# pedrocr/imagepipe

Hardware: AMD Instinct MI355X
Metric: megapixels/sec full raw->sRGB pipe, 100 MP f32 frame (higher is better)
Workload: dtype f32

## Files before the change

### bindings/rust/imagepipe_amd_sys.rs

```rust
#![allow(non_camel_case_types, dead_code)]
use std::os::raw::{c_char, c_int, c_uint, c_void};

pub const IPK_OK: c_int = 0;
pub const IPK_NOOP: c_int = 1;
pub const IPK_ERR_NOT_INIT: c_int = -1;
pub const IPK_ERR_INVALID: c_int = -2;
pub const IPK_ERR_HIP: c_int = -3;
pub const IPK_ERR_NO_DEVICE: c_int = -4;
pub const IPK_ERR_UNSUPPORTED: c_int = -5;
pub const IPK_ERR_NOMEM: c_int = -6;

pub const IPK_OR_NORMAL: c_int = 0;
pub const IPK_OR_HFLIP: c_int = 1;
pub const IPK_OR_ROT180: c_int = 2;
pub const IPK_OR_VFLIP: c_int = 3;
pub const IPK_OR_TRANSPOSE: c_int = 4;
pub const IPK_OR_ROT90: c_int = 5;
pub const IPK_OR_TRANSVERSE: c_int = 6;
pub const IPK_OR_ROT270: c_int = 7;
pub const IPK_OR_UNKNOWN: c_int = 8;

pub const IPK_ROT_NORMAL: c_int = 0;
pub const IPK_ROT_90: c_int = 1;
pub const IPK_ROT_180: c_int = 2;
// ... 167 lines not shown
  pub fn ipk_tolab(src4: *const f32, width: usize, height: usize, monochrome: c_int, wb_coeffs: *const f32, cam_to_xyz_normalized: *const f32, dst3: *mut f32, stream: *mut c_void) -> c_int;
  pub fn ipk_basecurve(src3: *const f32, width: usize, height: usize, exposure: f32, points: *const f32, npoints: c_int, dst3: *mut f32, stream: *mut c_void) -> c_int;
  pub fn ipk_fromlab(src3: *const f32, width: usize, height: usize, dst3: *mut f32, stream: *mut c_void) -> c_int;
  pub fn ipk_gamma(src: *const f32, width: usize, height: usize, colors: usize, linear: c_int, dst: *mut f32, stream: *mut c_void) -> c_int;
  pub fn ipk_rotate_buffer(src3: *const f32, width: usize, height: usize, orientation: c_int, dst3: *mut f32, out_width: *mut usize, out_height: *mut usize, stream: *mut c_void) -> c_int;
  pub fn ipk_rotate_image_u8(src3: *const u8, width: usize, height: usize, orientation: c_int, dst3: *mut u8, out_width: *mut usize, out_height: *mut usize, stream: *mut c_void) -> c_int;
  pub fn ipk_rotate_image_u16(src3: *const u16, width: usize, height: usize, orientation: c_int, dst3: *mut u16, out_width: *mut usize, out_height: *mut usize, stream: *mut c_void) -> c_int;
  pub fn ipk_transform(src3: *const f32, width: usize, height: usize, rotation: c_int, fliph: c_int, flipv: c_int, dst3: *mut f32, out_width: *mut usize, out_height: *mut usize, stream: *mut c_void) -> c_int;
  pub fn ipk_output8bit(src: *const f32, n: usize, dst: *mut u8, stream: *mut c_void) -> c_int;
  pub fn ipk_output16bit(src: *const f32, n: usize, dst: *mut u16, stream: *mut c_void) -> c_int;
  pub fn ipk_raw_to_srgb(p: *const IpkFusedParams, src: *const c_void, dst: *mut c_void, stream: *mut c_void) -> c_int;
  pub fn ipk_raw_to_srgb_batch(p: *const IpkFusedParams, srcs: *const *const c_void, dsts: *const *mut c_void, n: usize, stream: *mut c_void) -> c_int;
  pub fn ipk_raw_to_srgb_oriented(p: *const IpkFusedParams, src: *const c_void, orientation: c_int, dst: *mut c_void, out_width: *mut usize, out_height: *mut usize, stream: *mut c_void) -> c_int;
  pub fn ipk_raw_to_srgb_resampled(p: *const IpkFusedParams, src: *const c_void, tlx: i64, tly: i64, trx: i64, try_: i64, blx: i64, bly: i64, nwidth: usize, nheight: usize, dst: *mut c_void, stream: *mut c_void) -> c_int;
  pub fn ipk_raw_to_srgb_scaled(p: *const IpkFusedParams, src: *const c_void, nwidth: usize, nheight: usize, dst: *mut c_void, stream: *mut c_void) -> c_int;
  pub fn ipk_raw_to_srgb_resampled_window(p: *const IpkFusedParams, src: *const c_void, tlx: i64, tly: i64, trx: i64, try_: i64, blx: i64, bly: i64, nwidth: usize, nheight: usize, wx: usize, wy: usize, ww: usize, wh: usize, dst: *mut c_void, stream: *mut c_void) -> c_int;
  pub fn ipk_raw_to_srgb_scaled_window(p: *const IpkFusedParams, src: *const c_void, nwidth: usize, nheight: usize, wx: usize, wy: usize, ww: usize, wh: usize, dst: *mut c_void, stream: *mut c_void) -> c_int;
  pub fn ipk_transform_window_footprint(width: usize, height: usize, tlx: i64, tly: i64, trx: i64, try_: i64, blx: i64, bly: i64, nwidth: usize, nheight: usize, wx: usize, wy: usize, ww: usize, wh: usize, out4: *mut usize) -> c_int;
  pub fn ipk_pointwise_chain(src4: *const f32, width: usize, height: usize, monochrome: c_int, wb_coeffs: *const f32, cam_to_xyz_normalized: *const f32, exposure: f32, points: *const f32, npoints: c_int, linear: c_int, dst3: *mut f32, stream: *mut c_void) -> c_int;
  pub fn ipk_pointwise_chain_out(src4: *const f32, width: usize, height: usize, monochrome: c_int, wb_coeffs: *const f32, cam_to_xyz_normalized: *const f32, exposure: f32, points: *const f32, npoints: c_int, linear: c_int, out_type: c_int, dst: *mut c_void, stream: *mut c_void) -> c_int;
  pub fn ipk_raster_to_srgb(src: *const c_void, src_type: c_int, width: usize, height: usize, wb_coeffs: *const f32, cam_to_xyz_normalized: *const f32, exposure: f32, points: *const f32, npoints: c_int, linear: c_int, out_type: c_int, dst: *mut c_void, stream: *mut c_void) -> c_int;
  pub fn ipk_pipeline_sizes(d: *const IpkPipelineDesc, demosaic_w: *mut usize, demosaic_h: *mut usize, final_w: *mut usize, final_h: *mut usize) -> c_int;
  pub fn ipk_pipeline_run(d: *const IpkPipelineDesc, src: *const c_void, dst: *mut c_void, out_type: c_int, used_fused: *mut c_int, stream: *mut c_void) -> c_int;
  pub fn ipk_pipeline_takes_fastpath(d: *const IpkPipelineDesc, out_type: c_int) -> c_int;
  pub fn ipk_pipeline_fuses_rotatecrop(d: *const IpkPipelineDesc, out_type: c_int) -> c_int;
  pub fn ipk_pipeline_fuses_scaledown(d: *const IpkPipelineDesc, out_type: c_int) -> c_int;
  pub fn ipk_pipeline_fuses_four_colour(d: *const IpkPipelineDesc, out_type: c_int) -> c_int;
  pub fn ipk_timing_begin() -> c_int;
  pub fn ipk_timing_end(out: *mut IpkStageTime, max_stages: c_int, n_stages: *mut c_int) -> c_int;
  pub fn ipk_host_pipeline_run(d: *const IpkPipelineDesc, src: *const c_void, dst: *mut c_void, out_type: c_int, used_fused: *mut c_int) -> c_int;
  pub fn ipk_pipeline_region(d: *const IpkPipelineDesc, out_type: c_int, x: usize, y: usize, w: usize, h: usize, src_x: *mut usize, src_y: *mut usize, src_w: *mut usize, src_h: *mut usize) -> c_int;
  pub fn ipk_pipeline_run_region(d: *const IpkPipelineDesc, src: *const c_void, x: usize, y: usize, w: usize, h: usize, dst: *mut c_void, out_type: c_int, windowed: *mut c_int, stream: *mut c_void) -> c_int;
  pub fn ipk_host_pipeline_run_region(d: *const IpkPipelineDesc, src: *const c_void, x: usize, y: usize, w: usize, h: usize, dst: *mut c_void, out_type: c_int, windowed: *mut c_int) -> c_int;
  pub fn ipk_host_pipeline_run_batch(d: *const IpkPipelineDesc, srcs: *const *const c_void, dsts: *const *mut c_void, n: usize, out_type: c_int, used_fused: *mut c_int) -> c_int;
  pub fn ipk_pipeline_run_batch(d: *const IpkPipelineDesc, srcs: *const *const c_void, dsts: *const *mut c_void, n: usize, out_type: c_int, used_fused: *mut c_int, stream: *mut c_void) -> c_int;
  pub fn ipk_pipeline_run_batch_multi(d: *const IpkPipelineDesc, srcs: *const *const c_void, dsts: *const *mut c_void, n: usize, out_type: c_int, used_fused: *mut c_int) -> c_int;
  pub fn ipk_devices_sync() -> c_int;
  pub fn ipk_host_pipeline_run_batch_multi(d: *const IpkPipelineDesc, srcs: *const *const c_void, dsts: *const *mut c_void, n: usize, out_type: c_int, used_fused: *mut c_int) -> c_int;
  pub fn ipk_host_alloc(bytes: usize) -> *mut c_void;
  pub fn ipk_host_free(p: *mut c_void);
  pub fn ipk_pipeline_hashes(d: *const IpkPipelineDesc, out_type: c_int, source_id: u64, out256: *mut u8) -> c_int;
  pub fn ipk_cache_new(max_bytes: usize, out: *mut *mut IpkCache) -> c_int;
  pub fn ipk_cache_free(cache: *mut IpkCache) -> c_int;
  pub fn ipk_cache_clear(cache: *mut IpkCache) -> c_int;
  pub fn ipk_cache_contains(cache: *const IpkCache, key32: *const u8) -> c_int;
  pub fn ipk_cache_stats(cache: *const IpkCache, bytes: *mut usize, entries: *mut usize, hits: *mut u64, misses: *mut u64, evictions: *mut u64) -> c_int;
  pub fn ipk_cache_get(cache: *mut IpkCache, key32: *const u8, data: *mut *const f32, width: *mut usize, height: *mut usize, colors: *mut usize, monochrome: *mut c_int) -> c_int;
  pub fn ipk_pipeline_run_cached(d: *const IpkPipelineDesc, src: *const c_void, source_id: u64, cache: *mut IpkCache, out_type: c_int, dst: *mut c_void, ops_run: *mut c_int, used_fused: *mut c_int, stream: *mut c_void) -> c_int;
  pub fn ipk_band_plan(height: usize, nranks: c_int, cfa_period: c_int, bands: *mut IpkBand) -> c_int;
  pub fn ipk_band_plan_scaled(height: usize, nheight: usize, nranks: c_int, bands: *mut IpkBand) -> c_int;
  pub fn ipk_raw_scaled_demosaic_band(src: *const c_void, src_type: c_int, owidth: usize, x: usize, width: usize, height: usize, black0: f32, white0: f32, cfa: *const c_char, nwidth: usize, nheight: usize, band: *const IpkBand, dst4: *mut f32, stream: *mut c_void) -> c_int;
  pub fn ipk_comm_unique_id(id128: *mut u8) -> c_int;
  pub fn ipk_comm_init_rccl(id128: *const u8, rank: c_int, nranks: c_int, out: *mut *mut IpkComm) -> c_int;
  pub fn ipk_comm_init_host(rank: c_int, nranks: c_int, exchange: IpkExchangeFn, ctx: *mut c_void, out: *mut *mut IpkComm) -> c_int;
  pub fn ipk_comm_free(comm: *mut IpkComm) -> c_int;
  pub fn ipk_comm_info(comm: *const IpkComm, rank: *mut c_int, nranks: *mut c_int, transport: *mut c_int) -> c_int;
  pub fn ipk_band_exchange_halo(comm: *mut IpkComm, slab: *mut c_void, row_bytes: usize, bands: *const IpkBand, stream: *mut c_void) -> c_int;
  pub fn ipk_host_band_exchange_halo(comm: *mut IpkComm, slab: *mut c_void, row_bytes: usize, bands: *const IpkBand) -> c_int;
  pub fn ipk_band_gather(comm: *mut IpkComm, frame: *mut c_void, out_row_bytes: usize, bands: *const IpkBand, root: c_int, stream: *mut c_void) -> c_int;
  pub fn ipk_host_band_gather(comm: *mut IpkComm, frame: *mut c_void, out_row_bytes: usize, bands: *const IpkBand, root: c_int) -> c_int;
  pub fn ipk_band_gather_begin(comm: *mut IpkComm, frame: *mut c_void, out_row_bytes: usize, bands: *const IpkBand, root: c_int, after_stream: *mut c_void) -> c_int;
  pub fn ipk_comm_wait(comm: *mut IpkComm, stream: *mut c_void) -> c_int;
  pub fn ipk_comm_selftest(comm: *mut IpkComm) -> c_int;
  pub fn ipk_host_gofloat_cfa_u16(src: *const u16, owidth: usize, oheight: usize, x: usize, y: usize, width: usize, height: usize, black0: f32, white0: f32, dst: *mut f32) -> c_int;
  pub fn ipk_host_gofloat_cfa_f32(src: *const f32, owidth: usize, oheight: usize, x: usize, y: usize, width: usize, height: usize, black0: f32, white0: f32, dst: *mut f32) -> c_int;
  pub fn ipk_host_demosaic_full(src: *const f32, width: usize, height: usize, cfa: *const c_char, dst4: *mut f32) -> c_int;
  pub fn ipk_host_transform_buffer_f32(src: *const f32, width: usize, height: usize, tlx: i64, tly: i64, trx: i64, try_: i64, blx: i64, bly: i64, nwidth: usize, nheight: usize, components: usize, cfa: *const c_char, dst: *mut f32) -> c_int;
  pub fn ipk_host_tolab(src4: *const f32, width: usize, height: usize, monochrome: c_int, wb_coeffs: *const f32, cam_to_xyz_normalized: *const f32, dst3: *mut f32) -> c_int;
  pub fn ipk_host_basecurve(src3: *const f32, width: usize, height: usize, exposure: f32, points: *const f32, npoints: c_int, dst3: *mut f32) -> c_int;
  pub fn ipk_host_fromlab(src3: *const f32, width: usize, height: usize, dst3: *mut f32) -> c_int;
  pub fn ipk_host_gamma(src: *const f32, width: usize, height: usize, colors: usize, linear: c_int, dst: *mut f32) -> c_int;
  pub fn ipk_host_rotate_buffer(src3: *const f32, width: usize, height: usize, orientation: c_int, dst3: *mut f32, out_width: *mut usize, out_height: *mut usize) -> c_int;
  pub fn ipk_host_output8bit(src: *const f32, n: usize, dst: *mut u8) -> c_int;
  pub fn ipk_host_output16bit(src: *const f32, n: usize, dst: *mut u16) -> c_int;
  pub fn ipk_host_raw_to_srgb(p: *const IpkFusedParams, src: *const c_void, dst: *mut c_void) -> c_int;
  pub fn ipk_selftest_cdiv(c: f32, variant: c_int, lo: f32, hi: f32, include_special: c_int, n_bad: *mut u64, first_bad_bits: *mut u32) -> c_int;
  pub fn ipk_selftest_lut_weight(n_bad: *mut u64, first_bad_bits: *mut u32) -> c_int;
  pub fn ipk_selftest_clamp01(n_bad: *mut u64, first_bad_bits: *mut u32) -> c_int;
  pub fn ipk_copy_probe(src: *const c_void, dst: *mut c_void, bytes: usize, stream: *mut c_void) -> c_int;
  pub fn ipk_mix_probe(src: *const c_void, dst: *mut c_void, src_bytes: usize, stream: *mut c_void) -> c_int;
  pub fn ipk_clock_probe(out2_dev: *mut u64, spin_us: u32, stream: *mut c_void) -> c_int;
  pub fn ipk_stream_probe(p: *const IpkFusedParams, src: *const c_void, dst: *mut c_void, stream: *mut c_void) -> c_int;
  pub fn ipk_selftest_spline3(exposure: f32, points: *const f32, npoints: c_int, n_bad: *mut u64, first_bad_bits: *mut u32) -> c_int;
  pub fn ipk_selftest_quant8(variant: c_int, n_bad: *mut u64, first_bad_bits: *mut u32) -> c_int;
  pub fn ipk_selftest_q8(n_bad: *mut u64, first_bad_bits: *mut u32) -> c_int;
  pub fn ipk_selftest_quant16(n_bad: *mut u64, first_bad_bits: *mut u32) -> c_int;
  pub fn ipk_selftest_cbrtf(r#in: *const f32, out: *mut f32, n: usize, variant: c_int, stream: *mut c_void) -> c_int;
  pub fn ipk_selftest_task_queue(enabled: c_int) -> c_int;
  pub fn ipk_selftest_launch_log(enabled: c_int) -> c_int;
  pub fn ipk_selftest_launch_log_read(buf: *mut c_char, cap: usize) -> usize;
  pub fn ipk_selftest_cache_put(cache: *mut IpkCache, key32: *const u8, bytes: usize) -> c_int;
  pub fn ipk_selftest_sha256(data: *const c_void, n: usize, out32: *mut u8) -> c_int;
}
```

### imagepipe_amd/_lib.py

```python
import ctypes as C
import os

_HERE = os.path.dirname(os.path.abspath(__file__))
SO_PATH = os.environ.get("IPK_SO_OVERRIDE") or os.path.join(_HERE, "libimagepipe_amd.so")

IPK_OK, IPK_NOOP = 0, 1
SRC_U16, SRC_F32, SRC_RGB8, SRC_RGB16 = 0, 1, 2, 3
OUT_F32, OUT_U8, OUT_U16 = 0, 1, 2
SCHED_AUTO, SCHED_SPLIT = 0, 1
FUSED_ON, FUSED_FOUR_COLOUR, FUSED_WINDOW_REGIONS = 1, 2, 4
OR_NORMAL, OR_HFLIP, OR_ROT180, OR_VFLIP, OR_TRANSPOSE, OR_ROT90, OR_TRANSVERSE, OR_ROT270, OR_UNKNOWN = range(9)
ROT_NORMAL, ROT_90, ROT_180, ROT_270 = range(4)

_sz = C.c_size_t
_vp = C.c_void_p
_fp = C.POINTER(C.c_float)
_szp = C.POINTER(C.c_size_t)
_i64 = C.c_int64


class _SizedDesc(C.Structure):

    def __init__(self, *a, **k):
        super().__init__(*a, **k)
# ... 73 lines not shown
    "ipk_orientation_to_flips": (C.c_int, [C.c_int, C.POINTER(C.c_int)]),
    "ipk_orientation_from_flips": (C.c_int, [C.c_int, C.c_int, C.c_int]),
    "ipk_transform_orientation": (C.c_int, [C.c_int, C.c_int, C.c_int]),
    "ipk_gofloat_cfa_u16": (C.c_int, [_vp] + _GO + [C.c_float, C.c_float, _vp, _vp]),
    "ipk_gofloat_cfa_f32": (C.c_int, [_vp] + _GO + [C.c_float, C.c_float, _vp, _vp]),
    "ipk_gofloat_mono_u16": (C.c_int, [_vp] + _GO + [C.c_float, C.c_float, _vp, _vp]),
    "ipk_gofloat_mono_f32": (C.c_int, [_vp] + _GO + [C.c_float, C.c_float, _vp, _vp]),
    "ipk_gofloat_rgb_u16": (C.c_int, [_vp] + _GO + [_fp, _fp, _vp, _vp]),
    "ipk_gofloat_rgb_f32": (C.c_int, [_vp] + _GO + [_fp, _fp, _vp, _vp]),
    "ipk_gofloat_other_u8": (C.c_int, [_vp] + _GO + [_vp, _vp]),
    "ipk_gofloat_other_u16": (C.c_int, [_vp] + _GO + [_vp, _vp]),
    "ipk_demosaic_full": (C.c_int, [_vp, _sz, _sz, C.c_char_p, _vp, _vp]),
    "ipk_demosaic_full_band": (C.c_int, [_vp, _sz, _sz, _sz, _sz, _sz, _sz, C.c_char_p, _vp, _vp]),
    "ipk_transform_buffer_f32": (C.c_int, [_vp, _sz, _sz] + _CORNERS + [_sz, _sz, _sz, C.c_char_p, _vp, _vp]),
    "ipk_transform_buffer_u8": (C.c_int, [_vp, _sz, _sz] + _CORNERS + [_sz, _sz, _sz, C.c_char_p, _vp, _vp]),
    "ipk_transform_buffer_u16": (C.c_int, [_vp, _sz, _sz] + _CORNERS + [_sz, _sz, _sz, C.c_char_p, _vp, _vp]),
    "ipk_scaled_demosaic": (C.c_int, [_vp, _sz, _sz, C.c_char_p, _sz, _sz, _vp, _vp]),
    "ipk_scale_down_opbuf": (C.c_int, [_vp, _sz, _sz, _sz, _sz, _vp, _vp]),
    "ipk_raw_scaled_demosaic": (C.c_int, [_vp, C.c_int, _sz, _sz, _sz, _sz, _sz, C.c_float, C.c_float, C.c_char_p, _sz, _sz, _vp, _vp]),
    "ipk_raster_scale_down": (C.c_int, [_vp, C.c_int, _sz, _sz, _sz, _sz, _sz, _sz, _sz, _vp, _vp]),
    "ipk_demosaic_run": (C.c_int, [_vp, _sz, _sz, _sz, C.c_char_p, _sz, _sz, _vp, _szp, _szp, _vp]),
    "ipk_rotatecrop": (C.c_int, [_vp, _sz, _sz, _sz, _fp, _vp, _szp, _szp, _vp]),
    "ipk_tolab": (C.c_int, [_vp, _sz, _sz, C.c_int, _fp, _fp, _vp, _vp]),
    "ipk_basecurve": (C.c_int, [_vp, _sz, _sz, C.c_float, _fp, C.c_int, _vp, _vp]),
    "ipk_fromlab": (C.c_int, [_vp, _sz, _sz, _vp, _vp]),
    "ipk_gamma": (C.c_int, [_vp, _sz, _sz, _sz, C.c_int, _vp, _vp]),
    "ipk_rotate_buffer": (C.c_int, [_vp, _sz, _sz, C.c_int, _vp, _szp, _szp, _vp]),
    "ipk_rotate_image_u8": (C.c_int, [_vp, _sz, _sz, C.c_int, _vp, _szp, _szp, _vp]),
    "ipk_rotate_image_u16": (C.c_int, [_vp, _sz, _sz, C.c_int, _vp, _szp, _szp, _vp]),
    "ipk_transform": (C.c_int, [_vp, _sz, _sz, C.c_int, C.c_int, C.c_int, _vp, _szp, _szp, _vp]),
    "ipk_output8bit": (C.c_int, [_vp, _sz, _vp, _vp]),
    "ipk_output16bit": (C.c_int, [_vp, _sz, _vp, _vp]),
    "ipk_raw_to_srgb": (C.c_int, [C.POINTER(FusedParams), _vp, _vp, _vp]),
    "ipk_raw_to_srgb_batch": (C.c_int, [C.POINTER(FusedParams), C.POINTER(C.c_void_p), C.POINTER(C.c_void_p), _sz, _vp]),
    "ipk_raw_to_srgb_oriented": (C.c_int, [C.POINTER(FusedParams), _vp, C.c_int, _vp, _szp, _szp, _vp]),
    "ipk_raw_to_srgb_resampled": (C.c_int, [C.POINTER(FusedParams), _vp] + _CORNERS + [_sz, _sz, _vp, _vp]),
    "ipk_raw_to_srgb_scaled": (C.c_int, [C.POINTER(FusedParams), _vp, _sz, _sz, _vp, _vp]),
    "ipk_raw_to_srgb_resampled_window": (C.c_int, [C.POINTER(FusedParams), _vp] + _CORNERS + [_sz, _sz, _sz, _sz, _sz, _sz, _vp, _vp]),
    "ipk_raw_to_srgb_scaled_window": (C.c_int, [C.POINTER(FusedParams), _vp, _sz, _sz, _sz, _sz, _sz, _sz, _vp, _vp]),
    "ipk_transform_window_footprint": (C.c_int, [_sz, _sz] + _CORNERS + [_sz, _sz, _sz, _sz, _sz, _sz, _szp]),
    "ipk_pipeline_sizes": (C.c_int, [C.POINTER(PipelineDesc), _szp, _szp, _szp, _szp]),
    "ipk_pipeline_run": (C.c_int, [C.POINTER(PipelineDesc), _vp, _vp, C.c_int, C.POINTER(C.c_int), _vp]),
    "ipk_host_pipeline_run": (C.c_int, [C.POINTER(PipelineDesc), _vp, _vp, C.c_int, C.POINTER(C.c_int)]),
    "ipk_pipeline_region": (C.c_int, [C.POINTER(PipelineDesc), C.c_int, _sz, _sz, _sz, _sz, _szp, _szp, _szp, _szp]),
    "ipk_pipeline_run_region": (C.c_int, [C.POINTER(PipelineDesc), _vp, _sz, _sz, _sz, _sz, _vp, C.c_int, C.POINTER(C.c_int), _vp]),
    "ipk_host_pipeline_run_region": (C.c_int, [C.POINTER(PipelineDesc), _vp, _sz, _sz, _sz, _sz, _vp, C.c_int, C.POINTER(C.c_int)]),
    "ipk_host_pipeline_run_batch": (C.c_int, [C.POINTER(PipelineDesc), C.POINTER(_vp), C.POINTER(_vp), _sz, C.c_int, C.POINTER(C.c_int)]),
    "ipk_pipeline_run_batch": (C.c_int, [C.POINTER(PipelineDesc), C.POINTER(_vp), C.POINTER(_vp), _sz, C.c_int, C.POINTER(C.c_int), _vp]),
    "ipk_pipeline_run_batch_multi": (C.c_int, [C.POINTER(PipelineDesc), C.POINTER(_vp), C.POINTER(_vp), _sz, C.c_int, C.POINTER(C.c_int)]),
    "ipk_host_pipeline_run_batch_multi": (C.c_int, [C.POINTER(PipelineDesc), C.POINTER(_vp), C.POINTER(_vp), _sz, C.c_int, C.POINTER(C.c_int)]),
    "ipk_devices_sync": (C.c_int, []),
    "ipk_ctx_create": (C.c_int, [C.c_int, C.POINTER(_vp)]),
    "ipk_ctx_destroy": (C.c_int, [_vp]),
    "ipk_ctx_make_current": (C.c_int, [_vp]),
    "ipk_ctx_current": (_vp, []),
    "ipk_ctx_device": (C.c_int, [_vp]),
    "ipk_init_devices": (C.c_int, [C.POINTER(C.c_int), C.c_int]),
    "ipk_device_set_size": (C.c_int, []),
    "ipk_device_ctx": (_vp, [C.c_int]),
    "ipk_deal_frames": (C.c_int, [_sz, C.c_int, C.c_int, _szp, _szp, _szp]),
    "ipk_host_alloc": (_vp, [_sz]),
    "ipk_host_free": (None, [_vp]),
    "ipk_host_gofloat_cfa_u16": (C.c_int, [_vp, _sz, _sz, _sz, _sz, _sz, _sz, C.c_float, C.c_float, _vp]),
    "ipk_host_gofloat_cfa_f32": (C.c_int, [_vp, _sz, _sz, _sz, _sz, _sz, _sz, C.c_float, C.c_float, _vp]),
    "ipk_host_demosaic_full": (C.c_int, [_vp, _sz, _sz, C.c_char_p, _vp]),
    "ipk_host_transform_buffer_f32": (C.c_int, [_vp, _sz, _sz] + _CORNERS + [_sz, _sz, _sz, C.c_char_p, _vp]),
    "ipk_host_tolab": (C.c_int, [_vp, _sz, _sz, C.c_int, _fp, _fp, _vp]),
    "ipk_host_basecurve": (C.c_int, [_vp, _sz, _sz, C.c_float, _fp, C.c_int, _vp]),
    "ipk_host_fromlab": (C.c_int, [_vp, _sz, _sz, _vp]),
    "ipk_host_gamma": (C.c_int, [_vp, _sz, _sz, _sz, C.c_int, _vp]),
    "ipk_host_rotate_buffer": (C.c_int, [_vp, _sz, _sz, C.c_int, _vp, _szp, _szp]),
    "ipk_host_output8bit": (C.c_int, [_vp, _sz, _vp]),
    "ipk_host_output16bit": (C.c_int, [_vp, _sz, _vp]),
    "ipk_host_raw_to_srgb": (C.c_int, [C.POINTER(FusedParams), _vp, _vp]),
    "ipk_selftest_cdiv": (C.c_int, [C.c_float, C.c_int, C.c_float, C.c_float, C.c_int, C.POINTER(C.c_uint64), C.POINTER(C.c_uint32)]),
    "ipk_selftest_lut_weight": (C.c_int, [C.POINTER(C.c_uint64), C.POINTER(C.c_uint32)]),
    "ipk_selftest_clamp01": (C.c_int, [C.POINTER(C.c_uint64), C.POINTER(C.c_uint32)]),
    "ipk_abi_sizeof": (_sz, [C.c_int]),
    "ipk_copy_probe": (C.c_int, [_vp, _vp, _sz, _vp]),
    "ipk_mix_probe": (C.c_int, [_vp, _vp, _sz, _vp]),
    "ipk_clock_probe": (C.c_int, [_vp, C.c_uint32, _vp]),
    "ipk_stream_probe": (C.c_int, [C.POINTER(FusedParams), _vp, _vp, _vp]),
    "ipk_selftest_spline3": (C.c_int, [C.c_float, _fp, C.c_int, C.POINTER(C.c_uint64), C.POINTER(C.c_uint32)]),
    "ipk_selftest_quant8": (C.c_int, [C.c_int, C.POINTER(C.c_uint64), C.POINTER(C.c_uint32)]),
    "ipk_selftest_q8": (C.c_int, [C.POINTER(C.c_uint64), C.POINTER(C.c_uint32)]),
    "ipk_selftest_quant16": (C.c_int, [C.POINTER(C.c_uint64), C.POINTER(C.c_uint32)]),
    "ipk_selftest_cbrtf": (C.c_int, [_vp, _vp, _sz, C.c_int, _vp]),
    "ipk_selftest_task_queue": (C.c_int, [C.c_int]),
    "ipk_selftest_launch_log": (C.c_int, [C.c_int]),
    "ipk_selftest_launch_log_read": (_sz, [C.c_char_p, _sz]),
    "ipk_selftest_cache_put": (C.c_int, [_vp, C.c_char_p, _sz]),
    "ipk_selftest_sha256": (C.c_int, [C.c_char_p, _sz, C.c_char_p]),
    "ipk_pointwise_chain": (C.c_int, [_vp, _sz, _sz, C.c_int, _fp, _fp, C.c_float, _fp, C.c_int, C.c_int, _vp, _vp]),
    "ipk_pointwise_chain_out": (C.c_int, [_vp, _sz, _sz, C.c_int, _fp, _fp, C.c_float, _fp, C.c_int, C.c_int, C.c_int, _vp, _vp]),
    "ipk_raster_to_srgb": (C.c_int, [_vp, C.c_int, _sz, _sz, _fp, _fp, C.c_float, _fp, C.c_int, C.c_int, C.c_int, _vp, _vp]),
    "ipk_pipeline_takes_fastpath": (C.c_int, [C.POINTER(PipelineDesc), C.c_int]),
    "ipk_pipeline_fuses_rotatecrop": (C.c_int, [C.POINTER(PipelineDesc), C.c_int]),
    "ipk_pipeline_fuses_scaledown": (C.c_int, [C.POINTER(PipelineDesc), C.c_int]),
    "ipk_pipeline_fuses_four_colour": (C.c_int, [C.POINTER(PipelineDesc), C.c_int]),
    "ipk_pipeline_hashes": (C.c_int, [C.POINTER(PipelineDesc), C.c_int, C.c_uint64, C.c_char_p]),
    "ipk_cache_new": (C.c_int, [_sz, C.POINTER(C.c_void_p)]),
    "ipk_cache_free": (C.c_int, [_vp]),
    "ipk_cache_clear": (C.c_int, [_vp]),
    "ipk_cache_contains": (C.c_int, [_vp, C.c_char_p]),
    "ipk_cache_stats": (C.c_int, [_vp, C.POINTER(_sz), C.POINTER(_sz), C.POINTER(C.c_uint64), C.POINTER(C.c_uint64), C.POINTER(C.c_uint64)]),
    "ipk_cache_get": (C.c_int, [_vp, C.c_char_p, C.POINTER(C.c_void_p), C.POINTER(_sz), C.POINTER(_sz), C.POINTER(_sz), C.POINTER(C.c_int)]),
    "ipk_timing_begin": (C.c_int, []),
    "ipk_timing_end": (C.c_int, [C.POINTER(StageTime), C.c_int, C.POINTER(C.c_int)]),
    "ipk_band_plan": (C.c_int, [_sz, C.c_int, C.c_int, _bp]),
    "ipk_band_plan_scaled": (C.c_int, [_sz, _sz, C.c_int, _bp]),
    "ipk_raw_scaled_demosaic_band": (C.c_int, [_vp, C.c_int, _sz, _sz, _sz, _sz, C.c_float, C.c_float, C.c_char_p, _sz, _sz, _bp, _vp, _vp]),
    "ipk_comm_unique_id": (C.c_int, [C.c_char_p]),
    "ipk_comm_init_rccl": (C.c_int, [C.c_char_p, C.c_int, C.c_int, C.POINTER(_vp)]),
    "ipk_comm_init_host": (C.c_int, [C.c_int, C.c_int, EXCHANGE_FN, _vp, C.POINTER(_vp)]),
    "ipk_comm_free": (C.c_int, [_vp]),
    "ipk_comm_info": (C.c_int, [_vp, C.POINTER(C.c_int), C.POINTER(C.c_int), C.POINTER(C.c_int)]),
    "ipk_band_exchange_halo": (C.c_int, [_vp, _vp, _sz, _bp, _vp]),
    "ipk_host_band_exchange_halo": (C.c_int, [_vp, _vp, _sz, _bp]),
    "ipk_band_gather": (C.c_int, [_vp, _vp, _sz, _bp, C.c_int, _vp]),
    "ipk_host_band_gather": (C.c_int, [_vp, _vp, _sz, _bp, C.c_int]),
    "ipk_band_gather_begin": (C.c_int, [_vp, _vp, _sz, _bp, C.c_int, _vp]),
    "ipk_comm_wait": (C.c_int, [_vp, _vp]),
    "ipk_comm_selftest": (C.c_int, [_vp]),
    "ipk_pipeline_run_cached": (C.c_int, [C.POINTER(PipelineDesc), _vp, C.c_uint64, _vp, C.c_int, _vp, C.POINTER(C.c_int), C.POINTER(C.c_int), _vp]),
}

_lib = None


class IpkError(RuntimeError):
    code = None


def load():
    global _lib
    if _lib is not None:
        return _lib
    if not os.path.exists(SO_PATH):
        raise ImportError(
            "imagepipe_amd: %s is missing -- build it with `python -c 'import __graft_entry__ as g; g.build()'` "
            "or `make -C imagepipe_amd/csrc`. There is no CPU fallback." % SO_PATH)
    lib = C.CDLL(SO_PATH, mode=C.RTLD_GLOBAL)
    for name, (res, args) in SIGNATURES.items():
        if os.environ.get("IPK_SO_OVERRIDE") and not hasattr(lib, name):
            continue
        fn = getattr(lib, name)
        fn.restype = res
        fn.argtypes = args
    _lib = lib
    return lib


def check(rc, what=""):
    if rc < 0:
        err = IpkError("%s failed (%d): %s" % (what or "ipk call", rc, load().ipk_last_error().decode()))
        err.code = rc
        raise err
    return rc
```

### imagepipe_amd/csrc/ipk_api.cpp

```cpp
#include <hip/hip_runtime_api.h>

#include <algorithm>
#include <cmath>
#include <cstdarg>
#include <cstdio>
#include <cstddef>
#include <cstring>
#include <atomic>
#include <map>
#include <memory>
#include <mutex>
#include <string>
#include <thread>
#include <vector>

#include "../../include/imagepipe_amd.h"
#include "ipk_hash.hpp"
#include "ipk_host.hpp"
#include "ipk_internal.hpp"
#include "ipk_launch.hpp"

namespace {

thread_local char g_err[512] = "";
// ... 1166 lines not shown
  return resampled_launch(p, src, corners, nwidth, nheight, dst, stream, "resampled", kResampledRefusal, &win);
}
int ipk_raw_to_srgb_scaled_window(const ipk_fused_params *p, const void *src, size_t nwidth, size_t nheight, size_t wx, size_t wy, size_t ww, size_t wh,
                                  void *dst, void *stream) {
  const ipk::ResampleWindow win = {wy, wx, wh, ww};
  return resampled_launch(p, src, nullptr, nwidth, nheight, dst, stream, "scaled", kScaledRefusal, &win);
}
int ipk_transform_window_footprint(size_t width, size_t height, int64_t tlx, int64_t tly, int64_t trx, int64_t try_, int64_t blx, int64_t bly,
                                   size_t nwidth, size_t nheight, size_t wx, size_t wy, size_t ww, size_t wh, size_t *out4) {
  if (!out4) return fail(IPK_ERR_INVALID, "null argument");
  ipk::ResamplePlan plan;
  if (!ipk::resample_skips(width, height, tlx, tly, trx, try_, blx, bly, nwidth, nheight, plan))
    return fail(IPK_ERR_UNSUPPORTED, "not a transform the fused paths take (output sides >= 2, finite skips, sides below 2^24)");
  if (ww == 0 || wh == 0 || wx > nwidth || ww > nwidth - wx || wy > nheight || wh > nheight - wy)
    return fail(IPK_ERR_INVALID, "window (%zu, %zu) %zux%zu is empty or outside the %zux%zu result", wx, wy, ww, wh, nwidth, nheight);
  const ipk::ResampleFootprint f = ipk::resample_footprint(plan, width, height, wy, wx, wh, ww);
  out4[0] = f.x; out4[1] = f.y; out4[2] = f.w; out4[3] = f.h;
  return IPK_OK;
}

static int selftest_collect(void *dev, uint64_t *n_bad, uint32_t *first_bad) {
  struct { unsigned long long bad; unsigned int first; unsigned int pad; } h;
  HIPCHK(hipMemcpy(&h, dev, sizeof(h), hipMemcpyDeviceToHost));
  (void)hipFree(dev);
  *n_bad = h.bad; if (first_bad) *first_bad = h.first;
  return IPK_OK;
}
static int selftest_alloc(void **dev) {
  struct { unsigned long long bad; unsigned int first; unsigned int pad; } h = {0, 0xFFFFFFFFu, 0};
  HIPCHK(hipMalloc(dev, sizeof(h)));
  HIPCHK(hipMemcpy(*dev, &h, sizeof(h), hipMemcpyHostToDevice));
  return IPK_OK;
}
int ipk_selftest_cdiv(float c, int variant, float lo, float hi, int include_special, uint64_t *n_bad, uint32_t *first_bad_bits) {
  REQUIRE_INIT();
  if (!(c > 0.0f) || variant < 0 || variant > 2 || !n_bad) return fail(IPK_ERR_INVALID, "bad selftest arguments");
  uint32_t lo_bits, hi_bits; std::memcpy(&lo_bits, &lo, 4); std::memcpy(&hi_bits, &hi, 4);
  void *dev; int rc = selftest_alloc(&dev); if (rc) return rc;
  ipk::launch_selftest_cdiv(c, variant, lo_bits, hi_bits, include_special, dev, nullptr);
  HIPCHK(hipGetLastError());
  return selftest_collect(dev, n_bad, first_bad_bits);
}
int ipk_selftest_lut_weight(uint64_t *n_bad, uint32_t *first_bad_bits) {
  REQUIRE_INIT();
  void *dev; int rc = selftest_alloc(&dev); if (rc) return rc;
  ipk::launch_selftest_fract(dev, nullptr); HIPCHK(hipGetLastError());
  return selftest_collect(dev, n_bad, first_bad_bits);
}
int ipk_selftest_clamp01(uint64_t *n_bad, uint32_t *first_bad_bits) {
  REQUIRE_INIT();
  void *dev; int rc = selftest_alloc(&dev); if (rc) return rc;
  ipk::launch_selftest_clamp(dev, nullptr); HIPCHK(hipGetLastError());
  return selftest_collect(dev, n_bad, first_bad_bits);
}
int ipk_copy_probe(const void *src, void *dst, size_t bytes, void *stream) {
  REQUIRE_INIT();
  if (!src || !dst || (bytes & 15) || ((uintptr_t)src & 15) || ((uintptr_t)dst & 15)) return fail(IPK_ERR_INVALID, "ipk_copy_probe wants 16-byte aligned buffers and a multiple of 16 bytes");
  ipk::launch_copy_probe(src, dst, bytes, cx().num_cus, S(stream)); HIPCHK(hipGetLastError());
  return IPK_OK;
}
int ipk_mix_probe(const void *src, void *dst, size_t src_bytes, void *stream) {
  REQUIRE_INIT();
  if (!src || !dst || (src_bytes & 4095) || ((uintptr_t)src & 15) || ((uintptr_t)dst & 15)) return fail(IPK_ERR_INVALID, "ipk_mix_probe wants 16-byte aligned buffers and a multiple of 4096 source bytes (whole blocks)");
  ipk::launch_mix_probe(src, dst, src_bytes, S(stream)); HIPCHK(hipGetLastError());
  return IPK_OK;
}
int ipk_clock_probe(uint64_t *out2_dev, uint32_t spin_us, void *stream) {
  REQUIRE_INIT();
  if (!out2_dev || spin_us == 0 || spin_us > 2000000u) return fail(IPK_ERR_INVALID, "ipk_clock_probe: null output or a spin outside (0, 2 s]");
  ipk::launch_clock_probe(out2_dev, (unsigned long long)spin_us * 100ull, S(stream)); HIPCHK(hipGetLastError());
  return IPK_OK;
}
int ipk_selftest_launch_log(int enabled) { ipk::launch_log_enable(enabled != 0); return IPK_OK; }
size_t ipk_selftest_launch_log_read(char *buf, size_t cap) { return ipk::launch_log_read(buf, cap); }
int ipk_selftest_task_queue(int enabled) { REQUIRE_INIT(); ipk::selftest_task_queue(enabled != 0); return IPK_OK; }
int ipk_selftest_spline3(float exposure, const float *points, int npoints, uint64_t *n_bad, uint32_t *first_bad_bits) {
  REQUIRE_INIT();
  if (!n_bad || (npoints > 0 && !points)) return fail(IPK_ERR_INVALID, "bad selftest arguments");
  ipk::Spline sp; int rc = build_curve(exposure, points, npoints, sp); if (rc) return rc;
  void *dev; rc = selftest_alloc(&dev); if (rc) return rc;
  if (ipk::launch_selftest_spline3(sp, dev, nullptr) != 0) { (void)hipFree(dev); return fail(IPK_ERR_UNSUPPORTED, "the kernels keep the select form for this curve"); }
  HIPCHK(hipGetLastError());
  return selftest_collect(dev, n_bad, first_bad_bits);
}
int ipk_selftest_quant16(uint64_t *n_bad, uint32_t *first_bad_bits) {
  REQUIRE_INIT();
  if (!n_bad) return fail(IPK_ERR_INVALID, "bad selftest arguments");
  void *dev; int rc = selftest_alloc(&dev); if (rc) return rc;
  ipk::launch_selftest_quant16(dev, nullptr); HIPCHK(hipGetLastError());
  return selftest_collect(dev, n_bad, first_bad_bits);
}
int ipk_selftest_q8(uint64_t *n_bad, uint32_t *first_bad_bits) {
  REQUIRE_INIT();
  if (!n_bad) return fail(IPK_ERR_INVALID, "bad selftest arguments");
  void *dev; int rc = selftest_alloc(&dev); if (rc) return rc;
  ipk::launch_selftest_q8(cx().lut_pairs[ipk::kLutGamma], cx().lut_q8, dev, nullptr); HIPCHK(hipGetLastError());
  return selftest_collect(dev, n_bad, first_bad_bits);
}
int ipk_selftest_quant8(int variant, uint64_t *n_bad, uint32_t *first_bad_bits) {
  REQUIRE_INIT();
  void *dev; int rc = selftest_alloc(&dev); if (rc) return rc;
  ipk::launch_selftest_quant8(dev, variant, nullptr); HIPCHK(hipGetLastError());
  return selftest_collect(dev, n_bad, first_bad_bits);
}
int ipk_selftest_cbrtf(const float *in, float *out, size_t n, int variant, void *stream) {
  REQUIRE_INIT();
  if (!in || !out || variant < 0 || variant > 5 || (variant >= 3 && n % 256 != 0)) return fail(IPK_ERR_INVALID, "bad selftest arguments");
  ipk::launch_selftest_cbrt(in, out, n, variant, cx().lut_pairs[ipk::kLutXyzLab], S(stream)); HIPCHK(hipGetLastError());
  return IPK_OK;
}

static ipk::RotateCrop rotatecrop_of(const ipk_pipeline_desc *d) {
  ipk::RotateCrop rc;
  rc.crop_top = d->rotatecrop[0]; rc.crop_right = d->rotatecrop[1]; rc.crop_bottom = d->rotatecrop[2];
  rc.crop_left = d->rotatecrop[3]; rc.rotation = d->rotatecrop[4];
  return rc;
}
static int pipeline_sizes_impl(const ipk_pipeline_desc *d, size_t *demosaic_w, size_t *demosaic_h, size_t *final_w, size_t *final_h,
                               ipk::RotateCrop *rc_state) {
  if (!d) return fail(IPK_ERR_INVALID, "null descriptor");
  if (d->rotation < 0 || d->rotation > 3) return fail(IPK_ERR_INVALID, "bad rotation");
  ipk::RotateCrop rc = rotatecrop_of(d);
  ipk::Rect r;
  if (!ipk::size_image(d->crop_top, d->crop_right, d->crop_bottom, d->crop_left, d->width, d->height, r))
    return fail(IPK_ERR_INVALID, "source smaller than 10x10");
  size_t w = r.width, h = r.height;
  rc.transform_forward(w, h, w, h);
  ipk::transform_forward(d->rotation, w, h, w, h);
  const ipk::Scaling s = ipk::calculate_scaling_total(w, h, d->maxwidth, d->maxheight);
  w = s.width; h = s.height;
  ipk::transform_forward(d->rotation, w, h, w, h);
  rc.transform_reverse(w, h, w, h);
  if (rc_state) *rc_state = rc;
  *demosaic_w = w; *demosaic_h = h;
  size_t pw = r.width, ph = r.height;
  if (ipk::calculate_scaling_total(pw, ph, w, h).scale > 1.0f) { pw = w; ph = h; }
  {
    int64_t pts[6]; size_t nw, nh;
    if (rotatecrop_of(d).corners(pw, ph, pts, nw, nh)) { pw = nw; ph = nh; }
  }
  {
    bool transpose, fx, fy;
    ipk::orientation_to_flips(ipk::transform_orientation(d->rotation, d->fliph != 0, d->flipv != 0), transpose, fx, fy);
    if (transpose) std::swap(pw, ph);
  }
  *final_w = pw; *final_h = ph;
  return IPK_OK;
}
int ipk_pipeline_sizes(const ipk_pipeline_desc *d, size_t *demosaic_w, size_t *demosaic_h, size_t *final_w, size_t *final_h) {
  IPK_FOLD_CFA(ipk_pipeline_desc, d)
  return pipeline_sizes_impl(d, demosaic_w, demosaic_h, final_w, final_h, nullptr);
}

static bool default_ops_other(const ipk_pipeline_desc *d) {
  auto same = [](float a, float b) { return std::memcmp(&a, &b, 4) == 0; };
  if (d->src_type != IPK_SRC_RGB8 && d->src_type != IPK_SRC_RGB16) return false;
  if (d->crop_top || d->crop_right || d->crop_bottom || d->crop_left || d->is_cfa || d->cfa[0]) return false;
  for (int i = 0; i < 4; ++i) if (!same(d->blacklevels[i], 0.0f) || !same(d->whitelevels[i], 0.0f)) return false;
  for (int i = 0; i < 5; ++i) if (!same(d->rotatecrop[i], 0.0f)) return false;
  float m[12]; ipk::srgb_d65_43(m);
  for (int i = 0; i < 12; ++i) if (!same(d->cam_to_xyz_normalized[i], m[i])) return false;
  const float wb[4] = {1.0f, 1.0f, 1.0f, 0.0f};
  for (int i = 0; i < 4; ++i) if (!same(d->wb_coeffs[i], wb[i])) return false;
  if (!same(d->exposure, 0.0f) || d->npoints != 0) return false;
  return d->rotation == 0 && !d->fliph && !d->flipv;
}
// ... 1015 lines not shown
```

### imagepipe_amd/csrc/ipk_device.hpp

```cpp
#pragma once
#include <hip/hip_runtime.h>
#include <stdint.h>

namespace ipkd {

typedef float2 LutPair;
constexpr int kLutPairs = 8192;
constexpr float kLutMaxF = 8191.0f;

constexpr float kWhiteX = 0.95047f, kWhiteY = 1.000f, kWhiteZ = 1.08883f;
constexpr float kLabE = 216.0f / 24389.0f;
constexpr float kLabK = 24389.0f / 27.0f;

__device__ __forceinline__ float rs_min(float a, float b) { return fminf(a, b); }
__device__ __forceinline__ float rs_max(float a, float b) { return fmaxf(a, b); }
__device__ __forceinline__ uint32_t f32_as_u32_sat(float f) { return __float2uint_rz(f); }

__device__ __forceinline__ LutPair lut_pair_at(const LutPair *__restrict__ tab, uint32_t key) { return tab[key]; }
__device__ __forceinline__ LutPair lut_pair_at(const float *__restrict__ tab, uint32_t key) {
  const float v1 = tab[key], v2 = tab[key + 1];
  return make_float2(v1, v2 - v1);
}
template <typename Tab>
__device__ __forceinline__ float lut_interp(const Tab *__restrict__ tab, float val) {
// ... 138 lines not shown
__device__ __forceinline__ uint32_t q8_sample(const Q8Entry *__restrict__ tab, float c ) {
  const Q8Entry e = tab[f32_as_u32_sat(c * kLutMaxF)];
  return e.k + (c >= e.t ? 1u : 0u);
}

__device__ __forceinline__ uint8_t output8bit_literal(float v) {
  return (uint8_t)f32_as_u32_sat(rs_min(rs_max(v * 256.0f, 0.0f), 255.0f));
}
__device__ __forceinline__ uint8_t output8bit(float v) { return output8bit_literal(v); }
__device__ __forceinline__ uint32_t output8bit_x4(float a, float b, float c, float d) {
  uint32_t w = __builtin_amdgcn_cvt_pk_u8_f32(floorf(a * 256.0f), 0u, 0u);
  w = __builtin_amdgcn_cvt_pk_u8_f32(floorf(b * 256.0f), 1u, w);
  w = __builtin_amdgcn_cvt_pk_u8_f32(floorf(c * 256.0f), 2u, w);
  return __builtin_amdgcn_cvt_pk_u8_f32(floorf(d * 256.0f), 3u, w);
}
__device__ __forceinline__ uint16_t output16bit_literal(float v) {
  return (uint16_t)f32_as_u32_sat(rs_min(rs_max(roundf(v * 65535.0f), 0.0f), 65535.0f));
}
__device__ __forceinline__ uint32_t output16bit_x2(float a, float b) {
  typedef unsigned short u16x2 __attribute__((ext_vector_type(2)));
  const u16x2 p = __builtin_amdgcn_cvt_pk_u16(f32_as_u32_sat(floorf(a * 65535.0f + 0.5f)), f32_as_u32_sat(floorf(b * 65535.0f + 0.5f)));
  return (uint32_t)p.x | ((uint32_t)p.y << 16);
}
__device__ __forceinline__ uint16_t output16bit(float v) { return (uint16_t)(output16bit_x2(v, 0.0f) & 0xFFFFu); }
__device__ __forceinline__ float input8bit(uint8_t v) { return (float)v / 255.0f; }
__device__ __forceinline__ float input16bit(uint16_t v) { return (float)v / 65535.0f; }

constexpr int kSplineMaxKnots = 66;
constexpr int kKnotSegRec = 5 * kSplineMaxKnots + 2;
constexpr int kKnotFloats = kKnotSegRec + 16;
struct SplineDev {
  int npoints, nseg;
  float px[kSplineMaxKnots], py[kSplineMaxKnots], c1[kSplineMaxKnots], c2[kSplineMaxKnots], c3[kSplineMaxKnots];
  int grid_ok; float grid_scale, grid_xl, grid_yl;
};
__device__ __forceinline__ float spline_poly(float y, float c1, float c2, float c3, float diff) {
  return y + c1 * diff + c2 * diff * diff + c3 * diff * diff * diff;
}
__device__ __forceinline__ float spline_interpolate(const SplineDev &s, float val) {
  const int np = s.npoints;
  if (np == 2) {
    if (val >= s.px[1]) return s.py[1];
    if (!(val > s.px[0])) return s.py[0];
    return spline_poly(s.py[0], s.c1[0], s.c2[0], s.c3[0], val - s.px[0]);
  }
  if (np == 3) {
    if (val >= s.px[2]) return s.py[2];
    if (!(val > s.px[0])) return s.py[0];
    const float x1 = s.px[1];
    if (x1 < val) return spline_poly(s.py[1], s.c1[1], s.c2[1], s.c3[1], val - x1);
    if (x1 > val) return spline_poly(s.py[0], s.c1[0], s.c2[0], s.c3[0], val - s.px[0]);
    return s.py[1];
  }
  if (val >= s.px[np - 1]) return s.py[np - 1];
  if (val <= s.px[0]) return s.py[0];
  int low = 0, high = s.nseg - 1;
  while (low <= high) {
    const int mid = (low + high) / 2;
    const float xhere = s.px[mid];
    if (xhere < val) low = mid + 1;
    else if (xhere > val) high = mid - 1;
    else return s.py[mid];
  }
  const int i = high > 0 ? high : 0;
  return spline_poly(s.py[i], s.c1[i], s.c2[i], s.c3[i], val - s.px[i]);
}

__device__ __forceinline__ float spline_interpolate_lds(const float *__restrict__ t, int np, int nseg, float val) {
  const float *px = t, *py = t + kSplineMaxKnots, *c1 = t + 2 * kSplineMaxKnots, *c2 = t + 3 * kSplineMaxKnots, *c3 = t + 4 * kSplineMaxKnots;
  if (val >= px[np - 1]) return py[np - 1];
  if (val <= px[0]) return py[0];
  int low = 0, high = nseg - 1;
  while (low <= high) {
    const int mid = (low + high) / 2;
    const float xhere = px[mid];
    if (xhere < val) low = mid + 1;
    else if (xhere > val) high = mid - 1;
    else return py[mid];
  }
  const int i = high > 0 ? high : 0;
  return spline_poly(py[i], c1[i], c2[i], c3[i], val - px[i]);
}

__device__ __forceinline__ float spline_interpolate_3a(const SplineDev &s, const float *__restrict__ lds_knots, float val) {
  const float x0 = s.px[0], x1 = s.px[1], x2 = s.px[2];
  const float v1 = fmaxf(val, x0);
  const bool up = v1 >= x1;
  const float *rec = lds_knots + kKnotSegRec + (up ? 8 : 0);
  const float4 q = *reinterpret_cast<const float4 *>(rec);
  const float r = spline_poly(q.y, q.z, q.w, rec[4], v1 - q.x);
  return (val >= x2) ? s.py[2] : r;
}
__device__ __forceinline__ float spline_interpolate_sel(const SplineDev &s, const float *__restrict__ lds_knots, float val) {
  const int np = s.npoints;
  if (np == 3) {
    const float x0 = s.px[0], x1 = s.px[1], x2 = s.px[2];
    const bool up = x1 < val, down = x1 > val;
    const int i = up ? 1 : 0;
    const float bx = lds_knots[i], by = lds_knots[kSplineMaxKnots + i];
    const float k1 = lds_knots[2 * kSplineMaxKnots + i], k2 = lds_knots[3 * kSplineMaxKnots + i], k3 = lds_knots[4 * kSplineMaxKnots + i];
    float r = spline_poly(by, k1, k2, k3, val - bx);
    r = (!up && !down) ? s.py[1] : r;
    r = !(val > x0) ? s.py[0] : r;
    r = (val >= x2) ? s.py[2] : r;
    return r;
  }
  if (np == 2) {
    float r = spline_poly(s.py[0], s.c1[0], s.c2[0], s.c3[0], val - s.px[0]);
    r = !(val > s.px[0]) ? s.py[0] : r;
    r = (val >= s.px[1]) ? s.py[1] : r;
    return r;
  }
  return spline_interpolate_lds(lds_knots, np, s.nseg, val);
}

constexpr int kGridCells = 256;
constexpr int kGridFloats = 2 * kGridCells + 8 * kSplineMaxKnots;
__device__ __host__ inline uint32_t spline_grid_cell(float v1, float x0, float scale) {
  const float t = (v1 - x0) * scale;
#if defined(__HIP_DEVICE_COMPILE__)
  const uint32_t c = __float2uint_rz(t);
#else
  const uint32_t c = !(t < 4294967296.0f) ? 0xFFFFFFFFu : (uint32_t)t;
#endif
  return c < (uint32_t)(kGridCells - 1) ? c : (uint32_t)(kGridCells - 1);
}
__device__ __forceinline__ void fill_grid(float *__restrict__ g, const SplineDev &s, int t) {
  if (t >= kGridCells) return;
  const float x0 = s.px[0];
  uint32_t base = 0u; float nx = __builtin_inff();
  for (int k = 1; k < s.nseg; ++k) {
    const uint32_t ck = spline_grid_cell(s.px[k], x0, s.grid_scale);
    if (ck < (uint32_t)t) base = (uint32_t)k;
    else if (ck == (uint32_t)t) nx = s.px[k];
  }
  g[2 * t] = __uint_as_float((2u * kGridCells + 8u * base) * 4u);
  g[2 * t + 1] = nx;
  if (t < s.nseg) {
    float *r = g + 2 * kGridCells + 8 * t;
    r[0] = s.px[t]; r[1] = s.py[t]; r[2] = s.c1[t]; r[3] = s.c2[t]; r[4] = s.c3[t]; r[5] = 0.0f; r[6] = 0.0f; r[7] = 0.0f;
  }
}
__device__ __forceinline__ float spline_interpolate_grid(const SplineDev &s, const float *__restrict__ g, float val) {
  const float x0 = s.px[0];
  const float v1 = fmaxf(val, x0);
  const uint32_t c = spline_grid_cell(v1, x0, s.grid_scale);
  const float2 ce = reinterpret_cast<const float2 *>(g)[c];
  const uint32_t off = __float_as_uint(ce.x) + (ce.y <= v1 ? 32u : 0u);
  const float *rec = reinterpret_cast<const float *>(reinterpret_cast<const char *>(g) + off);
  const float4 q = *reinterpret_cast<const float4 *>(rec);
  const float r = spline_poly(q.y, q.z, q.w, rec[4], v1 - q.x);
  return (val >= s.grid_xl) ? s.grid_yl : r;
}

__device__ __forceinline__ void fill_knots(float *__restrict__ lds, const SplineDev &s, int i) {
  if (i < kSplineMaxKnots) {
    lds[i] = s.px[i]; lds[kSplineMaxKnots + i] = s.py[i]; lds[2 * kSplineMaxKnots + i] = s.c1[i];
    lds[3 * kSplineMaxKnots + i] = s.c2[i]; lds[4 * kSplineMaxKnots + i] = s.c3[i];
  }
  if (i < 2) {
    float *r = lds + kKnotSegRec + 8 * i;
    r[0] = s.px[i]; r[1] = s.py[i]; r[2] = s.c1[i]; r[3] = s.c2[i]; r[4] = s.c3[i]; r[5] = 0.0f; r[6] = 0.0f; r[7] = 0.0f;
  }
}

__device__ __forceinline__ float cdiv_fast(float x, float c, float rc) {
  const float q0 = x * rc;
// ... 16 lines not shown
```

### imagepipe_amd/csrc/ipk_host.hpp

```cpp
#pragma once
#include <cmath>
#include <cstdint>
#include <cstddef>
#include <cstring>
#include <limits>
#include <map>
#include <mutex>
#include <string>
#include <vector>

namespace ipk {

inline size_t f32_to_usize(float f) {
  if (!(f > 0.0f)) return 0;
  if (f >= 18446744073709551616.0f) return std::numeric_limits<size_t>::max();
  return static_cast<size_t>(f);
}
inline int64_t f32_to_isize(float f) {
  if (f != f) return 0;
  if (f >= 9223372036854775808.0f) return std::numeric_limits<int64_t>::max();
  if (f <= -9223372036854775808.0f) return std::numeric_limits<int64_t>::min();
  return static_cast<int64_t>(f);
}

// ... 253 lines not shown
  0.000000, 0.000000, 0.000000, 0.000000, 0.000000, 0.000000, 0.000000, 0.000000, 0.000000,
};
}
inline double powi5(double a) { double r = 1.0; for (int b = 5;;) { if (b & 1) r *= a; b /= 2; if (b == 0) break; a *= a; } return r; }
inline void temp_to_xyz(float temp, float out[3]) {
  constexpr double C1 = 3.7417717905326694e-16, C2 = 0.014387773457709927;
  double x = 0.0, y = 0.0, z = 0.0;
  for (int i = 0; i < 81; ++i) {
    const double wl = double(380 + 5 * i) / 1.0e9;
    const double power = C1 / (powi5(wl) * (std::exp(C2 / (double(temp) * wl)) - 1.0));
    x += power * cie::CIE_XBAR[i]; y += power * cie::CIE_YBAR[i]; z += power * cie::CIE_ZBAR[i];
  }
  const double mx = std::fmax(std::fmax(x, y), z);
  out[0] = float(x / mx); out[1] = float(y / mx); out[2] = float(z / mx);
}
inline void xyz_to_temp(const float xyz[3], float &temp, float &tint) {
  float mn = 1000.0f, mx = 40000.0f; temp = 0.0f;
  float n[3] = {0.0f, 0.0f, 0.0f};
  while ((mx - mn) > 1.0f) {
    temp = (mx + mn) / 2.0f;
    temp_to_xyz(temp, n);
    if ((n[2] / n[0]) > (xyz[2] / xyz[0])) mx = temp; else mn = temp;
  }
  tint = (n[1] / n[0]) / (xyz[1] / xyz[0]);
}
inline void tolab_set_temp(const float xyz_to_cam[12], float temp, float tint, float wb[4]) {
  float t[3]; temp_to_xyz(temp, t);
  const float xyz[3] = {t[0], t[1] / tint, t[2]};
  float w[4];
  for (int i = 0; i < 4; ++i) {
    w[i] = 0.0f;
    for (int j = 0; j < 3; ++j) w[i] += xyz_to_cam[i * 3 + j] * xyz[j];
    w[i] = 1.0f / w[i];
  }
  normalize_wbs(w, wb);
}
inline void tolab_get_temp(const float cam_to_xyz[12], const float wb[4], float &temp, float &tint) {
  float xyz[3] = {0.0f, 0.0f, 0.0f};
  for (int i = 0; i < 3; ++i)
    for (int j = 0; j < 4; ++j) { const float mul = wb[j]; if (mul > 0.0f) xyz[i] += cam_to_xyz[i * 4 + j] / mul; }
  xyz_to_temp(xyz, temp, tint);
}

constexpr int kSplineMaxKnots = 66;
struct Spline {
  int npoints = 0, nseg = 0;
  float px[kSplineMaxKnots], py[kSplineMaxKnots], c1[kSplineMaxKnots], c2[kSplineMaxKnots], c3[kSplineMaxKnots];
  bool build(const float *p, int n) {
    if (n < 0 || n > kSplineMaxKnots - 2) return false;
    int np = 0;
    if (n == 0 || (p[0] > 0.0f && p[1] > 0.0f)) { px[np] = 0.0f; py[np] = 0.0f; ++np; }
    for (int i = 0; i < n; ++i) { px[np] = p[2 * i]; py[np] = p[2 * i + 1]; ++np; }
    if (n == 0 || (p[2 * (n - 1)] < 1.0f && p[2 * (n - 1) + 1] < 1.0f)) { px[np] = 1.0f; py[np] = 1.0f; ++np; }
    if (np < 2) return false;
    npoints = np;
    const int nd = np - 1;
    float dxs[kSplineMaxKnots], slopes[kSplineMaxKnots];
    for (int i = 0; i < nd; ++i) {
      const float dx = px[i + 1] - px[i], dy = py[i + 1] - py[i];
      dxs[i] = dx; slopes[i] = dy / dx;
    }
    int k = 0;
    c1[k++] = slopes[0];
    for (int i = 0; i < nd - 1; ++i) {
      const float m = slopes[i], next = slopes[i + 1];
      if (m * next <= 0.0f) c1[k++] = 0.0f;
      else {
        const float dx = dxs[i], dxnext = dxs[i + 1], common = dx + dxnext;
        c1[k++] = 3.0f * common / ((common + dxnext) / m + (common + dx) / next);
      }
    }
    c1[k++] = slopes[nd - 1];
    nseg = 0;
    for (int i = 0; i < k - 1; ++i) {
      const float a = c1[i], slope = slopes[i], invdx = 1.0f / dxs[i];
      const float common = a + c1[i + 1] - slope - slope;
      c2[nseg] = (slope - a - common) * invdx;
      c3[nseg] = common * invdx * invdx;
      ++nseg;
    }
    return true;
  }
};

inline void orientation_to_flips(int o, bool &transpose, bool &fx, bool &fy) {
  static const bool t[9][3] = {{0,0,0},{0,1,0},{0,1,1},{0,0,1},{1,0,0},{1,0,1},{1,1,1},{1,1,0},{0,0,0}};
  if (o < 0 || o > 8) o = 8;
  transpose = t[o][0]; fx = t[o][1]; fy = t[o][2];
}
inline int orientation_from_flips(bool transpose, bool fx, bool fy) {
  for (int o = 0; o < 8; ++o) { bool a, b, c; orientation_to_flips(o, a, b, c); if (a == transpose && b == fx && c == fy) return o; }
  return 8;
}
inline int transform_orientation(int rotation, bool fliph, bool flipv) {
  static const int base[4] = {0 , 5 , 2 , 7 };
  bool t, fx, fy; orientation_to_flips(base[rotation & 3], t, fx, fy);
  return orientation_from_flips(t, fx != fliph, fy != flipv);
}
inline void transform_forward(int rotation, size_t w, size_t h, size_t &ow, size_t &oh) {
  if (rotation == 1 || rotation == 3) { ow = h; oh = w; } else { ow = w; oh = h; }
}

struct RotateCrop {
  float crop_top = 0, crop_right = 0, crop_bottom = 0, crop_left = 0, rotation = 0;
  float input_ratio = 1.0f;
  bool has_output = false; size_t out_w = 0, out_h = 0;
  static constexpr float kEps = 1.0f / 1000000.0f;
  static constexpr float kFracPi2 = 1.57079632679489661923132169163975144f;

  void reset() { input_ratio = 1.0f; has_output = false; out_w = out_h = 0; }
  bool noop() const {
    return std::fabs(rotation) < kEps && std::fabs(crop_top) < kEps && std::fabs(crop_right) < kEps &&
           std::fabs(crop_bottom) < kEps && std::fabs(crop_left) < kEps;
  }
  float angle() const { return kFracPi2 * (rotation > 1.0f ? 1.0f : rotation); }
  void calc_size(size_t owidth, size_t oheight, bool reverse, size_t &rw, size_t &rh) const {
    rw = owidth; rh = oheight;
    if (noop()) return;
    float width = float(owidth), height = float(oheight);
    if (!(reverse || rotation < kEps)) {
      const float sn = std::sin(angle()), cs = std::cos(angle());
      const float w2 = width * cs + height * sn, h2 = width * sn + height * cs;
      width = w2; height = h2;
    }
    float nwidth, nheight;
    {
      const float ratio = 1.0f - crop_left - crop_right;
      nwidth = reverse ? std::round(width / ratio) : std::round(width * ratio);
      if (ratio < kEps || nwidth < 1.0f) return;
    }
    {
      const float ratio = 1.0f - crop_top - crop_bottom;
      nheight = reverse ? std::round(height / ratio) : std::round(height * ratio);
      if (ratio < kEps || nheight < 1.0f) return;
    }
    if (!(!reverse || rotation < kEps)) {
      const float sn = std::sin(angle()), cs = std::cos(angle());
      const float w2 = std::round(nheight / (sn + (cs / input_ratio)));
      const float h2 = std::round(w2 / input_ratio);
      nwidth = w2; nheight = h2;
    }
    rw = f32_to_usize(nwidth); rh = f32_to_usize(nheight);
  }
  void transform_forward(size_t w, size_t h, size_t &ow, size_t &oh) {
    if (has_output) { ow = out_w; oh = out_h; }
    else { input_ratio = float(w) / float(h); calc_size(w, h, false, ow, oh); }
  }
  void transform_reverse(size_t w, size_t h, size_t &ow, size_t &oh) {
    has_output = true; out_w = w; out_h = h;
    calc_size(w, h, true, ow, oh);
  }
  void rotate_point_reverse(float x, float y, float width, float height, float swidth, float sheight,
                            int64_t &ox, int64_t &oy) const {
    if (rotation < kEps) { ox = f32_to_isize(x); oy = f32_to_isize(y); return; }
    const float sn = std::sin(angle()), cs = std::cos(angle());
    const float tx = x - (width / 2.0f), ty = y - (height / 2.0f);
    const float nx = tx * cs + ty * sn + (swidth / 2.0f);
    const float ny = -tx * sn + ty * cs + (sheight / 2.0f);
    ox = f32_to_isize(nx); oy = f32_to_isize(ny);
  }
  bool corners(size_t width, size_t height, int64_t pts[6], size_t &nw, size_t &nh) const {
    if (noop()) return false;
    const float swidth = float(width), sheight = float(height);
    calc_size(width, height, false, nw, nh);
    const float fnw = float(nw), fnh = float(nh);
    const float x = std::floor(swidth * crop_left);
// ... 111 lines not shown
```

### imagepipe_amd/csrc/ipk_kernels.hip

```cpp
#include <hip/hip_runtime.h>
#include <stdint.h>
#include <cstring>
#include <cmath>
#include <type_traits>
#include <algorithm>
#include <atomic>
#include <mutex>
#include <set>
#include <string>
#include <utility>
#include <vector>
#include "ipk_device.hpp"
#include "ipk_launch.hpp"

using namespace ipkd;

#define IPK_RARE(x) __builtin_expect(!!(x), 0)
constexpr uint32_t kSpread = 4;
constexpr uint32_t kMinTaskRows = 4;
#ifndef IPK_SPLIT_MIN_ROWS
#define IPK_SPLIT_MIN_ROWS 16u
#endif
constexpr uint32_t kStealMin = 4;

// ... 949 lines not shown
  for (size_t i = (size_t)blockIdx.x * blockDim.x + threadIdx.x; i < n; i += (size_t)gridDim.x * blockDim.x) {
    const float *pi = reinterpret_cast<const float *>(src + i);
    float *po = reinterpret_cast<float *>(dst + i);
    const float l = ld_stream(pi), ca = ld_stream(pi + 1), cb = ld_stream(pi + 2);
    st_stream(po, spline_interpolate(sp, l)); st_stream(po + 1, ca); st_stream(po + 2, cb);
  }
}
__global__ void k_fromlab(const f3 *__restrict__ src, size_t n, Mat9 m, f3 *__restrict__ dst) {
  for (size_t i = (size_t)blockIdx.x * blockDim.x + threadIdx.x; i < n; i += (size_t)gridDim.x * blockDim.x) {
    const float *pi = reinterpret_cast<const float *>(src + i);
    float *po = reinterpret_cast<float *>(dst + i);
    const float l = ld_stream(pi), ca = ld_stream(pi + 1), cb = ld_stream(pi + 2);
    f3 o;
    lab_to_rgb(m, l, ca, cb, o.x, o.y, o.z);
    st_stream(po, o.x); st_stream(po + 1, o.y); st_stream(po + 2, o.z);
  }
}
__global__ __launch_bounds__(1024) void k_gamma(const float *__restrict__ src, size_t n, const LutPair *__restrict__ gam_pairs,
                                                float *__restrict__ dst) {
  __shared__ LutPair s_gam[kLutPairs];
  load_lut_pairs(s_gam, gam_pairs);
  __syncthreads();
  const size_t n4 = ((reinterpret_cast<uintptr_t>(src) | reinterpret_cast<uintptr_t>(dst)) & 15) == 0 ? n / 4 : 0;
  auto one = [&](size_t k, const float4 &v) {
    st_stream4(dst + 4 * k, make_float4(gamma_sample(s_gam, v.x), gamma_sample(s_gam, v.y), gamma_sample(s_gam, v.z), gamma_sample(s_gam, v.w)));
    __builtin_amdgcn_sched_barrier(0);
  };
  const size_t bs = 4 * (size_t)blockDim.x, gs = bs * gridDim.x;
  size_t j = (size_t)blockIdx.x * bs + threadIdx.x;
  for (; j + 3 * blockDim.x < n4; j += gs) {
    const float4 v0 = ld_stream4(src + 4 * j), v1 = ld_stream4(src + 4 * (j + blockDim.x)), v2 = ld_stream4(src + 4 * (j + 2 * blockDim.x)), v3 = ld_stream4(src + 4 * (j + 3 * blockDim.x));
    __builtin_amdgcn_sched_barrier(0);
    one(j, v0); one(j + blockDim.x, v1); one(j + 2 * blockDim.x, v2); one(j + 3 * blockDim.x, v3);
  }
  if (j < n4) {
    #pragma unroll
    for (int u = 0; u < 4; ++u) if (j + u * blockDim.x < n4) one(j + u * blockDim.x, ld_stream4(src + 4 * (j + u * blockDim.x)));
  }
  for (size_t i = 4 * n4 + (size_t)blockIdx.x * blockDim.x + threadIdx.x; i < n; i += (size_t)gridDim.x * blockDim.x)
    dst[i] = gamma_sample(s_gam, src[i]);
}
template <typename T> struct __attribute__((packed)) Px3 { T x, y, z; };
template <typename T>
__global__ void k_rotate(const Px3<T> *__restrict__ src, uint32_t owidth, uint32_t oheight, int64_t base_offset, int64_t x_step,
                         int64_t y_step, Px3<T> *__restrict__ dst) {
  const uint32_t col = blockIdx.x * blockDim.x + threadIdx.x;
  if (col >= owidth) return;
  for (uint32_t row = blockIdx.y; row < oheight; row += gridDim.y) {
    const int64_t offset = base_offset + y_step * (int64_t)row + x_step * (int64_t)col;
    dst[(size_t)row * owidth + col] = src[offset];
  }
}
__global__ void k_output8(const float *__restrict__ src, size_t n, uint8_t *__restrict__ dst) {
  const size_t n4 = ((reinterpret_cast<uintptr_t>(src) & 15) | (reinterpret_cast<uintptr_t>(dst) & 3)) == 0 ? n / 4 : 0;
  for (size_t i = (size_t)blockIdx.x * blockDim.x + threadIdx.x; i < n4; i += (size_t)gridDim.x * blockDim.x) {
    const float4 v = ld_stream4(src + 4 * i);
    st_stream_u(reinterpret_cast<uint32_t *>(dst) + i, output8bit_x4(v.x, v.y, v.z, v.w));
  }
  for (size_t i = 4 * n4 + (size_t)blockIdx.x * blockDim.x + threadIdx.x; i < n; i += (size_t)gridDim.x * blockDim.x) dst[i] = output8bit(src[i]);
}
__global__ void k_output16(const float *__restrict__ src, size_t n, uint16_t *__restrict__ dst) {
  const size_t n4 = ((reinterpret_cast<uintptr_t>(src) & 15) | (reinterpret_cast<uintptr_t>(dst) & 7)) == 0 ? n / 4 : 0;
  for (size_t i = (size_t)blockIdx.x * blockDim.x + threadIdx.x; i < n4; i += (size_t)gridDim.x * blockDim.x) {
    const float4 v = ld_stream4(src + 4 * i);
    st_stream_u(reinterpret_cast<uint32_t *>(dst) + 2 * i, output16bit_x2(v.x, v.y));
    st_stream_u(reinterpret_cast<uint32_t *>(dst) + 2 * i + 1, output16bit_x2(v.z, v.w));
  }
  for (size_t i = 4 * n4 + (size_t)blockIdx.x * blockDim.x + threadIdx.x; i < n; i += (size_t)gridDim.x * blockDim.x) dst[i] = output16bit(src[i]);
}

static ToLabParams make_tolab(const float *mul4, const float *cm12) {
  ToLabParams p;
  for (int i = 0; i < 4; ++i) p.mul[i] = mul4[i];
  for (int i = 0; i < 12; ++i) p.cm[i] = cm12[i];
  return p;
}
static bool spline3_arith_ok(const SplineDev &d) {
  for (int i = 0; i < 3; ++i) {
    if (!std::isfinite(d.px[i]) || !std::isfinite(d.py[i]) || (d.py[i] == 0.0f && std::signbit(d.py[i]))) return false;
    if (i < 2 && !(std::isfinite(d.c1[i]) && std::isfinite(d.c2[i]) && std::isfinite(d.c3[i]))) return false;
  }
  return true;
}
static bool spline_grid_ok(const SplineDev &d, float &scale) {
  if (d.npoints < 4 || d.npoints > kSplineMaxKnots || d.nseg != d.npoints - 1) return false;
  for (int i = 0; i < d.npoints; ++i) {
    if (!std::isfinite(d.px[i]) || !std::isfinite(d.py[i]) || (d.py[i] == 0.0f && std::signbit(d.py[i]))) return false;
    if (i > 0 && !(d.px[i] > d.px[i - 1])) return false;
    if (i < d.nseg && !(std::isfinite(d.c1[i]) && std::isfinite(d.c2[i]) && std::isfinite(d.c3[i]))) return false;
  }
  const float span = d.px[d.npoints - 1] - d.px[0];
  scale = (float)kGridCells / span;
  if (!(span > 0.0f) || !std::isfinite(scale) || !(scale > 0.0f)) return false;
  uint32_t prev = 0; bool have = false;
  for (int k = 1; k < d.nseg; ++k) {
    const uint32_t ck = spline_grid_cell(d.px[k], d.px[0], scale);
    if (have && ck <= prev) return false;
    prev = ck; have = true;
  }
  return true;
}
static SplineDev make_spline(const SplineHost &h) {
  SplineDev d;
  d.npoints = h.npoints; d.nseg = h.nseg;
  for (int i = 0; i < kSplineMaxKnots; ++i) { d.px[i] = h.px[i]; d.py[i] = h.py[i]; d.c1[i] = h.c1[i]; d.c2[i] = h.c2[i]; d.c3[i] = h.c3[i]; }
  d.grid_ok = 0; d.grid_scale = 0.0f; d.grid_xl = 0.0f; d.grid_yl = 0.0f;
  float scale;
  if (spline_grid_ok(d, scale)) { d.grid_ok = 1; d.grid_scale = scale; d.grid_xl = d.px[d.npoints - 1]; d.grid_yl = d.py[d.npoints - 1]; }
  return d;
}

void launch_tolab(const float *src4, size_t npix, const float *mul4, const float *cm12, const void *lab_pairs, float *dst3,
                  int num_cus, hipStream_t s) {
  IPK_LAUNCH(k_tolab, dim3(grid_1d(npix, 1024, (unsigned)num_cus * 2)), dim3(1024), 0, s,
                     reinterpret_cast<const float4 *>(src4), npix, make_tolab(mul4, cm12),
                     reinterpret_cast<const LutPair *>(lab_pairs), reinterpret_cast<f3 *>(dst3));
}
void launch_basecurve(const float *src3, size_t npix, const SplineHost &sp, float *dst3, int num_cus, hipStream_t s) {
  IPK_LAUNCH(k_basecurve, dim3(grid_1d(npix, 256, flat_cap((unsigned)num_cus * 16))), dim3(256), 0, s,
                     reinterpret_cast<const f3 *>(src3), npix, make_spline(sp), reinterpret_cast<f3 *>(dst3));
}
void launch_fromlab(const float *src3, size_t npix, const float *m9, float *dst3, int num_cus, hipStream_t s) {
  Mat9 m; for (int i = 0; i < 9; ++i) m.m[i] = m9[i];
  IPK_LAUNCH(k_fromlab, dim3(grid_1d(npix, 256, flat_cap((unsigned)num_cus * 16))), dim3(256), 0, s,
                     reinterpret_cast<const f3 *>(src3), npix, m, reinterpret_cast<f3 *>(dst3));
}
void launch_gamma(const float *src, size_t n, const void *gam_pairs, float *dst, int num_cus, hipStream_t s) {
  const bool vec4 = ((reinterpret_cast<uintptr_t>(src) | reinterpret_cast<uintptr_t>(dst)) & 15) == 0;
  const bool wrap = (n / 4 + 3) / 4 > (size_t)num_cus * 16 * 1024;
  IPK_LAUNCH_TAG(vec4 ? (wrap ? "vec4=1,wrap=1" : "vec4=1,wrap=0") : (wrap ? "vec4=0,wrap=1" : "vec4=0,wrap=0"),
                 k_gamma, dim3(grid_1d((n / 4 + 3) / 4, 1024, (unsigned)num_cus * 16)), dim3(1024), 0, s, src, n,
                     reinterpret_cast<const LutPair *>(gam_pairs), dst);
}
template <typename T>
__global__ __launch_bounds__(256) void k_rotate_transposed(const Px3<T> *__restrict__ src, uint32_t owidth, uint32_t oheight, int64_t base_offset,
                                                          int64_t x_step, int64_t y_step, Px3<T> *__restrict__ dst) {
  __shared__ T tile[32][33 * 3];
  const uint32_t C0 = blockIdx.x * 32, R0 = blockIdx.y * 32;
  const uint32_t a = threadIdx.x & 31u, b = threadIdx.x >> 5;
  #pragma unroll
  for (uint32_t i = 0; i < 4; ++i) {
    const uint32_t lr = a, lc = b + 8 * i;
    const uint32_t r = R0 + lr, c = C0 + lc;
    if (r < oheight && c < owidth) {
      const Px3<T> v = src[base_offset + y_step * (int64_t)r + x_step * (int64_t)c];
      tile[lc][3 * lr] = v.x; tile[lc][3 * lr + 1] = v.y; tile[lc][3 * lr + 2] = v.z;
    }
  }
  __syncthreads();
  #pragma unroll
  for (uint32_t i = 0; i < 4; ++i) {
    const uint32_t lc = a, lr = b + 8 * i;
    const uint32_t r = R0 + lr, c = C0 + lc;
    if (r < oheight && c < owidth) dst[(size_t)r * owidth + c] = Px3<T>{tile[lc][3 * lr], tile[lc][3 * lr + 1], tile[lc][3 * lr + 2]};
  }
}
template <typename T>
void launch_rotate(const T *src3, size_t owidth, size_t oheight, int64_t base_offset_px, int64_t x_step_px, int64_t y_step_px,
                   T *dst3, hipStream_t s) {
  if ((y_step_px == 1 || y_step_px == -1) && x_step_px != 1 && x_step_px != -1 && (oheight + 31) / 32 <= 65535) {
    IPK_LAUNCH(k_rotate_transposed<T>, dim3((unsigned)((owidth + 31) / 32), (unsigned)((oheight + 31) / 32), 1), dim3(256), 0, s,
                       reinterpret_cast<const Px3<T> *>(src3), (uint32_t)owidth, (uint32_t)oheight, base_offset_px, x_step_px, y_step_px,
                       reinterpret_cast<Px3<T> *>(dst3));
    return;
  }
  IPK_LAUNCH(k_rotate<T>, grid_rows(owidth, oheight, 256), dim3(256), 0, s, reinterpret_cast<const Px3<T> *>(src3),
// ... 556 lines not shown
  if (nvalid == 4) { const us4u t = *reinterpret_cast<const us4u *>(p); v0 = (float)t.x; v1 = (float)t.y; v2 = (float)t.z; v3 = (float)t.w; }
  else { v0 = nvalid > 0 ? (float)p[0] : 0.0f; v1 = nvalid > 1 ? (float)p[1] : 0.0f; v2 = nvalid > 2 ? (float)p[2] : 0.0f; v3 = 0.0f; }
}

template <int OUT> struct OutStore;
template <> struct OutStore<3> { static __device__ __forceinline__ void store(void *, size_t, uint32_t, const PixOut *, bool) {} };
template <> struct OutStore<0> {
  typedef float elem;
  static __device__ __forceinline__ void store(void *dst, size_t pix, uint32_t nvalid, const PixOut o[4], bool) {
    float *p = reinterpret_cast<float *>(dst) + pix * 3;
    if (nvalid == 4) {
      f4u a{o[0].r, o[0].g, o[0].b, o[1].r}, b{o[1].g, o[1].b, o[2].r, o[2].g}, c{o[2].b, o[3].r, o[3].g, o[3].b};
      reinterpret_cast<f4u *>(p)[0] = a; reinterpret_cast<f4u *>(p)[1] = b; reinterpret_cast<f4u *>(p)[2] = c;
    } else {
      #pragma unroll
      for (int j = 0; j < 3; ++j)
        if ((uint32_t)j < nvalid) { p[3 * j] = o[j].r; p[3 * j + 1] = o[j].g; p[3 * j + 2] = o[j].b; }
    }
  }
};
template <> struct OutStore<1> {
  typedef uint8_t elem;
  static __device__ __forceinline__ void store(void *dst, size_t pix, uint32_t nvalid, const PixOut o[4], bool aligned) {
    uint8_t *p = reinterpret_cast<uint8_t *>(dst) + pix * 3;
    uint8_t q[12];
    #pragma unroll
    for (int j = 0; j < 4; ++j) { q[3 * j] = output8bit(o[j].r); q[3 * j + 1] = output8bit(o[j].g); q[3 * j + 2] = output8bit(o[j].b); }
    if (nvalid == 4 && aligned) {
      u3w w;
      w.x = q[0] | (q[1] << 8) | (q[2] << 16) | ((uint32_t)q[3] << 24);
      w.y = q[4] | (q[5] << 8) | (q[6] << 16) | ((uint32_t)q[7] << 24);
      w.z = q[8] | (q[9] << 8) | (q[10] << 16) | ((uint32_t)q[11] << 24);
      *reinterpret_cast<u3w *>(p) = w;
    } else {
      #pragma unroll
      for (int j = 0; j < 12; ++j)
        if ((uint32_t)j < nvalid * 3) p[j] = q[j];
    }
  }
};
template <> struct OutStore<2> {
  typedef uint16_t elem;
  static __device__ __forceinline__ void store(void *dst, size_t pix, uint32_t nvalid, const PixOut o[4], bool aligned) {
    uint16_t *p = reinterpret_cast<uint16_t *>(dst) + pix * 3;
    uint16_t q[12];
    #pragma unroll
    for (int j = 0; j < 4; ++j) { q[3 * j] = output16bit(o[j].r); q[3 * j + 1] = output16bit(o[j].g); q[3 * j + 2] = output16bit(o[j].b); }
    if (nvalid == 4 && aligned) {
      uint32_t *pw = reinterpret_cast<uint32_t *>(p);
      #pragma unroll
      for (int j = 0; j < 6; ++j) pw[j] = q[2 * j] | ((uint32_t)q[2 * j + 1] << 16);
    } else {
      #pragma unroll
      for (int j = 0; j < 12; ++j)
        if ((uint32_t)j < nvalid * 3) p[j] = q[j];
    }
  }
};

template <int OUT> struct OutStage;
template <> struct OutStage<3> {
  static __device__ __forceinline__ void stage(uint32_t *, uint32_t, const PixOut *) {}
  static __device__ __forceinline__ void flush(const uint32_t *, uint32_t, void *, size_t) {}
};
template <> struct OutStage<0> {
  static __device__ __forceinline__ void stage(uint32_t *stg, uint32_t lane, const PixOut o[4]) {
    float4 *p = reinterpret_cast<float4 *>(stg + 12 * lane);
    p[0] = make_float4(o[0].r, o[0].g, o[0].b, o[1].r);
    p[1] = make_float4(o[1].g, o[1].b, o[2].r, o[2].g);
    p[2] = make_float4(o[2].b, o[3].r, o[3].g, o[3].b);
  }
  static __device__ __forceinline__ void flush(const uint32_t *stg, uint32_t lane, void *dst, size_t pix) {
    f4u *g = reinterpret_cast<f4u *>(reinterpret_cast<float *>(dst) + pix * 3);
    const float4 *s = reinterpret_cast<const float4 *>(stg);
    const float4 q0 = s[lane], q1 = s[64 + lane], q2 = s[128 + lane];
    typedef float f4a __attribute__((ext_vector_type(4), aligned(4)));
    f4a *gn = reinterpret_cast<f4a *>(reinterpret_cast<float *>(dst) + pix * 3);
    f4a v0, v1, v2;
    v0.x = q0.x; v0.y = q0.y; v0.z = q0.z; v0.w = q0.w; v1.x = q1.x; v1.y = q1.y; v1.z = q1.z; v1.w = q1.w; v2.x = q2.x; v2.y = q2.y; v2.z = q2.z; v2.w = q2.w;
    { __builtin_nontemporal_store(v0, gn + lane); __builtin_nontemporal_store(v1, gn + 64 + lane); __builtin_nontemporal_store(v2, gn + 128 + lane); }
    (void)g;
  }
};
template <> struct OutStage<1> {
  static __device__ __forceinline__ void stage_bits(uint32_t *stg, uint32_t lane, const PixOut o[4]) {
    auto B = [](float f) { return __float_as_uint(f); };
    uint32_t *p = stg + 3 * lane;
    p[0] = (B(o[0].r) | (B(o[0].g) << 8)) | ((B(o[0].b) | (B(o[1].r) << 8)) << 16);
    p[1] = (B(o[1].g) | (B(o[1].b) << 8)) | ((B(o[2].r) | (B(o[2].g) << 8)) << 16);
    p[2] = (B(o[2].b) | (B(o[3].r) << 8)) | ((B(o[3].g) | (B(o[3].b) << 8)) << 16);
  }
  static __device__ __forceinline__ void stage(uint32_t *stg, uint32_t lane, const PixOut o[4]) {
    uint32_t *p = stg + 3 * lane;
    p[0] = output8bit_x4(o[0].r, o[0].g, o[0].b, o[1].r);
    p[1] = output8bit_x4(o[1].g, o[1].b, o[2].r, o[2].g);
    p[2] = output8bit_x4(o[2].b, o[3].r, o[3].g, o[3].b);
  }
  static __device__ __forceinline__ void flush(const uint32_t *stg, uint32_t lane, void *dst, size_t pix) {
    u32u *g = reinterpret_cast<u32u *>(reinterpret_cast<uint8_t *>(dst) + pix * 3);
    const uint32_t q0 = stg[lane], q1 = stg[64 + lane], q2 = stg[128 + lane];
    typedef uint32_t u32a __attribute__((aligned(1)));
    u32a *gn = reinterpret_cast<u32a *>(reinterpret_cast<uint8_t *>(dst) + pix * 3);
    __builtin_nontemporal_store(q0, gn + lane); __builtin_nontemporal_store(q1, gn + 64 + lane); __builtin_nontemporal_store(q2, gn + 128 + lane);
    (void)g;
  }
};
template <> struct OutStage<2> {
  static __device__ __forceinline__ void stage(uint32_t *stg, uint32_t lane, const PixOut o[4]) {
    uint2 *p = reinterpret_cast<uint2 *>(stg + 6 * lane);
    p[0] = make_uint2(output16bit_x2(o[0].r, o[0].g), output16bit_x2(o[0].b, o[1].r));
    p[1] = make_uint2(output16bit_x2(o[1].g, o[1].b), output16bit_x2(o[2].r, o[2].g));
    p[2] = make_uint2(output16bit_x2(o[2].b, o[3].r), output16bit_x2(o[3].g, o[3].b));
  }
  static __device__ __forceinline__ void flush(const uint32_t *stg, uint32_t lane, void *dst, size_t pix) {
    u64u *g = reinterpret_cast<u64u *>(reinterpret_cast<uint16_t *>(dst) + pix * 3);
    const uint2 *s = reinterpret_cast<const uint2 *>(stg);
    const uint2 q0 = s[lane], q1 = s[64 + lane], q2 = s[128 + lane];
    typedef uint32_t u2a __attribute__((ext_vector_type(2), aligned(2)));
    u2a *gn = reinterpret_cast<u2a *>(reinterpret_cast<uint16_t *>(dst) + pix * 3);
    u2a v0, v1, v2; v0.x = q0.x; v0.y = q0.y; v1.x = q1.x; v1.y = q1.y; v2.x = q2.x; v2.y = q2.y;
    __builtin_nontemporal_store(v0, gn + lane); __builtin_nontemporal_store(v1, gn + 64 + lane); __builtin_nontemporal_store(v2, gn + 128 + lane);
    (void)g;
  }
};

struct RgbeStage {
  static __device__ __forceinline__ void stage(uint32_t *stg, uint32_t lane, const float4 px[4]) {
    float4 *p = reinterpret_cast<float4 *>(stg + 16 * lane);
    p[0] = px[0]; p[1] = px[1]; p[2] = px[2]; p[3] = px[3];
  }
  static __device__ __forceinline__ void flush(const uint32_t *stg, uint32_t lane, void *dst, size_t pix) {
    f4u *g = reinterpret_cast<f4u *>(reinterpret_cast<float *>(dst) + pix * 4);
    const float4 *s = reinterpret_cast<const float4 *>(stg);
    const float4 q0 = s[lane], q1 = s[64 + lane], q2 = s[128 + lane], q3 = s[192 + lane];
    g[lane] = f4u{q0.x, q0.y, q0.z, q0.w}; g[64 + lane] = f4u{q1.x, q1.y, q1.z, q1.w}; g[128 + lane] = f4u{q2.x, q2.y, q2.z, q2.w}; g[192 + lane] = f4u{q3.x, q3.y, q3.z, q3.w};
  }
  static __device__ __forceinline__ void store_direct(void *dst, size_t pix, uint32_t nvalid, const float4 px[4]) {
    float4 *g = reinterpret_cast<float4 *>(dst) + pix;
    #pragma unroll
    for (int j = 0; j < 4; ++j)
      if ((uint32_t)j < nvalid) g[j] = px[j];
  }
};

constexpr int kBatchMax = 64;
struct BatchPtrs { const void *src[kBatchMax]; void *dst[kBatchMax]; };
struct FusedWindow { uint32_t x0, x1, c0, c1; uint64_t pitch; };
template <int OUT, bool BITS>
__device__ __forceinline__ void win_store(void *dst, size_t rowpix, uint32_t col0, uint32_t c0, uint32_t c1, const PixOut o[4]) {
  const int64_t e = ((int64_t)rowpix + (int64_t)col0 - (int64_t)c0) * 3;
  #pragma unroll
  for (int j = 0; j < 4; ++j) {
    const uint32_t c = col0 + j;
    if (c < c0 || c >= c1) continue;
    if (OUT == 0) { float *p = reinterpret_cast<float *>(dst) + e + 3 * j; p[0] = o[j].r; p[1] = o[j].g; p[2] = o[j].b; }
    else if (OUT == 1) {
      uint8_t *p = reinterpret_cast<uint8_t *>(dst) + e + 3 * j;
      if (BITS) { p[0] = (uint8_t)__float_as_uint(o[j].r); p[1] = (uint8_t)__float_as_uint(o[j].g); p[2] = (uint8_t)__float_as_uint(o[j].b); }
      else { p[0] = output8bit(o[j].r); p[1] = output8bit(o[j].g); p[2] = output8bit(o[j].b); }
    } else { uint16_t *p = reinterpret_cast<uint16_t *>(dst) + e + 3 * j; p[0] = output16bit(o[j].r); p[1] = output16bit(o[j].g); p[2] = output16bit(o[j].b); }
  }
}
template <typename SrcT, bool VEC, int OUT, bool FULL, bool GEN, bool PXG, int CM, bool ROT, bool BATCH, bool WIN = false>
__device__ __forceinline__ void fused_bayer_body(const FusedArgs &a, const BatchPtrs *bp, const FusedWindow *win = nullptr) {
  constexpr bool CMN = CM != 0;
  constexpr bool DEMO = OUT == 3;
  constexpr bool SKEL = OUT == 4;
  constexpr int OUTS = SKEL ? 0 : OUT;
  constexpr bool ZA = DEMO;
  constexpr bool GUARD_NORM = sizeof(SrcT) == 4 && !DEMO;
  typedef typename std::conditional<GEN, float, LabTab>::type LabT;
  constexpr bool Q8 = OUTS == 1 && FULL && !GEN && !DEMO && !SKEL;
  typedef typename std::conditional<Q8, Q8Entry, typename std::conditional<GEN || OUTS == 0, float, GamTab>::type>::type GamT;
  __shared__ __attribute__((aligned(16))) LabT s_lab[DEMO ? 4 : kLutPairs + 4];
  __shared__ __attribute__((aligned(16))) GamT s_gam[DEMO ? 4 : kLutPairs + 4];
  if (!DEMO) {
    stage_table_direct(s_lab, a.lab_table, a.lab_pairs);
    if constexpr (Q8) stage_q8_direct(s_gam, a.gam_q8); else stage_table_direct(s_gam, a.gam_table, a.gam_pairs);
  }
  __shared__ __attribute__((aligned(16))) float s_knots[kKnotFloats];
  __shared__ float s_par[32];
  __shared__ __attribute__((aligned(16))) float s_cells[GEN ? kGenMaxCells * kGenCellFloats : 4];
  if (GEN) for (uint32_t i = threadIdx.x; i < a.gen_pw * a.gen_ph * kGenCellFloats; i += blockDim.x) s_cells[i] = a.gen_cells[i];
  constexpr bool FOUR_CAPABLE = GEN && CM == 0 && !ROT && !BATCH && !DEMO && !SKEL;
  float *e4 = nullptr;
  if constexpr (FOUR_CAPABLE) { __shared__ float s_e4[4 * 1024]; e4 = s_e4 + threadIdx.x; }
  constexpr int STG = DEMO ? 1024 : (OUTS == 0 ? 768 : (OUTS == 1 ? 192 : 384));
  __shared__ __attribute__((aligned(16))) uint32_t s_stage[FULL ? 16 * STG : 4];
  if (threadIdx.x < 4) s_par[threadIdx.x] = a.tolab.mul[threadIdx.x];
  else if (threadIdx.x < 16) s_par[threadIdx.x] = a.tolab.cm[threadIdx.x - 4];
  else if (threadIdx.x < 25) s_par[threadIdx.x] = a.rgbm.m[threadIdx.x - 16];
  if (threadIdx.x < kSplineMaxKnots) fill_knots(s_knots, a.spline, (int)threadIdx.x);
  constexpr bool HAS_GRID = CM != 1 && !DEMO && !SKEL;
  __shared__ __attribute__((aligned(16))) float s_grid[HAS_GRID ? kGridFloats : 4];
  if (HAS_GRID && (CM == 2 || a.spline.grid_ok)) fill_grid(s_grid, a.spline, (int)threadIdx.x);
  __shared__ unsigned long long s_tdesc[16];
  __shared__ uint32_t s_tcur[16];
  if ((threadIdx.x & 63u) == 0) { s_tdesc[threadIdx.x >> 6] = 0ull; s_tcur[threadIdx.x >> 6] = 0u; }
  bool arrived = false;
  auto arrive = [&]() { if (!arrived) { sync_after_lds_direct(); arrived = true; } };

  const uint32_t lane = threadIdx.x & 63u;
  const uint32_t per_frame = a.n_strips * a.n_segs;
  const uint32_t n_waves = gridDim.x * (blockDim.x >> 6);
  const uint32_t n_tasks = BATCH ? per_frame * a.n_frames : per_frame;
  auto draw = [&]() -> uint32_t {
    uint32_t t = 0xFFFFFFFFu;
    if ((threadIdx.x & 63u) == 0) {
      t = n_waves + atomicAdd(a.task_ctr, 1u);
    }
    t = (uint32_t)__builtin_amdgcn_readfirstlane((int)t);
    return t;
  };
  const bool queued = a.task_ctr != nullptr && n_tasks > n_waves;
  const uint32_t wslot = threadIdx.x >> 6, nwb = blockDim.x >> 6;
  const bool steal_on = a.n_strips <= 0xFFFFu && (!BATCH || a.n_frames <= 64u);
  uint32_t tserial = 0;
  auto take_over = [&](uint32_t &frame, uint32_t &strip, uint32_t &r0, uint32_t &r1) -> bool {
    for (int attempt = 0; attempt < 4; ++attempt) {
      unsigned long long d = 0ull; uint32_t c = 0u;
      if (lane < nwb) {
        d = __hip_atomic_load(&s_tdesc[lane], __ATOMIC_RELAXED, __HIP_MEMORY_SCOPE_WORKGROUP);
        c = __hip_atomic_load(&s_tcur[lane], __ATOMIC_RELAXED, __HIP_MEMORY_SCOPE_WORKGROUP);
      }
      const uint32_t e = (uint32_t)d;
      const uint32_t rem = e > c + 1u ? e - c - 1u : 0u;
      uint32_t best = 0u, bl = 0u;
      for (uint32_t i = 0; i < 16u; ++i) { const uint32_t x = (uint32_t)__builtin_amdgcn_readlane((int)rem, (int)i); if (x > best) { best = x; bl = i; } }
      if (best < kStealMin) return false;
      const uint32_t dlo = (uint32_t)__builtin_amdgcn_readlane((int)(uint32_t)d, (int)bl), dhi = (uint32_t)__builtin_amdgcn_readlane((int)(uint32_t)(d >> 32), (int)bl);
      const uint32_t mid = dlo - best / 2u;
      const unsigned long long dv = ((unsigned long long)dhi << 32) | dlo, nv = ((unsigned long long)dhi << 32) | mid;
      uint32_t ok = 0u;
      if (lane == 0) ok = atomicCAS(&s_tdesc[bl], dv, nv) == dv ? 1u : 0u;
      if (__builtin_amdgcn_readfirstlane((int)ok) != 0) { strip = dhi & 0xFFFFu; frame = (dhi >> 16) & 63u; r0 = mid; r1 = dlo; return true; }
    }
    return false;
  };
  const uint32_t gt0 = queued ? blockIdx.x * (blockDim.x >> 6) + (threadIdx.x >> 6)
                              : (((threadIdx.x >> 6) / kSpread) * gridDim.x + blockIdx.x) * kSpread + ((threadIdx.x >> 6) % kSpread);
  auto next_task = [&](uint32_t gt) -> uint32_t {
    if (gt >= n_tasks) return 0xFFFFFFFFu;
    if (queued) return draw();
    return (n_tasks - gt > n_waves) ? gt + n_waves : 0xFFFFFFFFu;
  };
  for (uint32_t gt = (uint32_t)__builtin_amdgcn_readfirstlane((int)gt0);; gt = next_task(gt)) {
    uint32_t frame = 0u, strip, r0, r1;
    if (gt < n_tasks) {
      frame = BATCH ? (uint32_t)__builtin_amdgcn_readfirstlane((int)(gt / per_frame)) : 0u;
      const uint32_t task = (uint32_t)__builtin_amdgcn_readfirstlane((int)(BATCH ? gt - frame * per_frame : gt));
      strip = task % a.n_strips;
      const uint32_t seg = task / a.n_strips;
      const uint32_t nrows = a.out_r1 - a.out_r0;
      r0 = a.out_r0 + (uint32_t)(((uint64_t)seg * nrows) / a.n_segs);
      r1 = a.out_r0 + (uint32_t)(((uint64_t)(seg + 1) * nrows) / a.n_segs);
    } else {
      arrive();
      if (!steal_on) break;
      if (lane == 0) __hip_atomic_store(&s_tdesc[wslot], (unsigned long long)(++tserial & 0x3FFu) << 54, __ATOMIC_RELAXED, __HIP_MEMORY_SCOPE_WORKGROUP);
      if (__builtin_amdgcn_readfirstlane(take_over(frame, strip, r0, r1) ? 1 : 0) == 0) break;
    }
    strip = (uint32_t)__builtin_amdgcn_readfirstlane((int)strip); r0 = (uint32_t)__builtin_amdgcn_readfirstlane((int)r0); r1 = (uint32_t)__builtin_amdgcn_readfirstlane((int)r1);
    if (BATCH) frame = (uint32_t)__builtin_amdgcn_readfirstlane((int)frame);
    const void *const frame_src = BATCH ? bp->src[frame] : a.src;
    void *const frame_dst = BATCH ? bp->dst[frame] : a.dst;

    const uint32_t lc0 = FULL ? 0u : strip * a.lc_base + min(strip, a.lc_rem);
    const uint32_t nl = FULL ? 64u : a.lc_base + (strip < a.lc_rem ? 1u : 0u);
    const bool lane_on = FULL ? true : lane < nl;
    const uint32_t pc0 = (WIN ? win->x0 : 0u) + (FULL ? min(strip * 256u, (WIN ? win->x1 - win->x0 : a.W) - 256u) : 4u * lc0);
// ... 158 lines not shown
              const float t[9] = {pw[j], pw[j + 1], pw[j + 2], cw[j], cw[j + 1], cw[j + 2], nw[j], nw[j + 1], nw[j + 2]};
              uint32_t m = 0x1FFu;
              if (r == 0) m &= ~0x007u;
              if (r == Hm1) m &= ~0x1C0u;
              if (c == 0) m &= ~0x049u;
              if (c == Wm1) m &= ~0x124u;
              if (ROT) {
                float to[9];
                const uint32_t mo = ori_window_dyn(a.ori, pw, cw, nw, j, to, m);
                const int role = a.roles[2 * (int)(r & 1u) + (int)((j + xo) & 1u)];
                px[j] = GEN ? demosaic_gen_literal_px(__float_as_uint(rowcells[cxo[j] + 27]), to, mo) : demosaic_edge_dispatch(to, mo, role >> 1, role & 1);
              } else
              px[j] = GEN ? demosaic_gen_literal_px(__float_as_uint(rowcells[cxo[j] + 27]), t, m) : demosaic_edge_dispatch(t, m, pr, (int)((j + xo) & 1u));
            }
          }
        }
      }
      if constexpr (FOUR_CAPABLE) if (IPK_RARE(four)) {
        #pragma unroll
        for (int j = 0; j < 4; ++j) {
          const uint32_t c = col0 + j;
          const float t[9] = {pw[j], pw[j + 1], pw[j + 2], cw[j], cw[j + 1], cw[j + 2], nw[j], nw[j + 1], nw[j + 2]};
          uint32_t m = 0x1FFu;
          if (r == 0) m &= ~0x007u;
          if (r == Hm1) m &= ~0x1C0u;
          if (c == 0) m &= ~0x049u;
          if (c == Wm1) m &= ~0x124u;
          const float4 q = demosaic_gen_literal_px<4>(__float_as_uint(rowcells[cxo[j] + 27]), t, m);
          e4[1024 * j] = q.w;
          px[j] = make_float4(q.x, q.y, q.z, 0.0f);
        }
      }
    };
    auto row_step = [&](RowWin &P, RowWin &C, RowWin &N, bool &fP, bool &fC, bool &fN, const uint32_t r) {
      if (!queued) switch ((r - r0) & 3u) {
        case 0: __builtin_amdgcn_s_setprio(3); break;
        case 1: __builtin_amdgcn_s_setprio(2); break;
        case 2: __builtin_amdgcn_s_setprio(1); break;
        default: __builtin_amdgcn_s_setprio(0); break;
      }
      float4 px[4];
      compute_px(P, C, N, fP, fC, fN, r, px);
      if (DEMO) {
        bool fNN;
        const RowWin NN = finish_row(raw_next, fNN);
        __builtin_amdgcn_sched_barrier(0);
        if (FULL) {
          uint32_t *stg = s_stage + (threadIdx.x >> 6) * STG;
          RgbeStage::stage(stg, lane, px);
          __builtin_amdgcn_fence(__ATOMIC_RELEASE, "wavefront"); __builtin_amdgcn_wave_barrier(); __builtin_amdgcn_fence(__ATOMIC_ACQUIRE, "wavefront");
          RgbeStage::flush(stg, lane, frame_dst, (size_t)(r - a.out_r0) * a.W + pc0);
          __builtin_amdgcn_fence(__ATOMIC_RELEASE, "wavefront"); __builtin_amdgcn_wave_barrier(); __builtin_amdgcn_fence(__ATOMIC_ACQUIRE, "wavefront");
        } else if (lane_on) {
          RgbeStage::store_direct(frame_dst, (size_t)(r - a.out_r0) * a.W + col0, nvalid, px);
        }
        __builtin_amdgcn_sched_barrier(0);
        raw_next = issue_row(min(r + 3, Hm1));
        P = NN; fP = fNN;
        if (GEN) ry = (ry + 1 == a.gen_ph) ? 0u : ry + 1;
        return;
      }
      PixOut o[4];
      if (SKEL) {
        #pragma unroll
        for (int j = 0; j < 4; ++j) { o[j].r = px[j].x; o[j].g = px[j].y; o[j].b = px[j].z; }
      } else {
      bool bad = !fast_ok || (!PXG && sizeof(SrcT) == 4 && (fP | fC | fN));
      if (fast_ok) bad |= pointwise4_fast<PXG>(a, s_par, s_lab, s_gam, s_knots, px, o, has_curve, linear, CM, nullptr, HAS_GRID ? s_grid : nullptr);
      if (IPK_RARE(__builtin_amdgcn_ballot_w64(bad) != 0)) {
        #pragma unroll
        for (int j = 0; j < 4; ++j) {
          float4 p = px[j];
          if constexpr (FOUR_CAPABLE) { if (four) p.w = e4[1024 * j]; }
          const PixOut e = pointwise_exact(a, s_lab, s_gam, s_knots, p);
          if (bad) o[j] = e;
        }
      }
      }
      bool fNN;
      const RowWin NN = finish_row(raw_next, fNN);
      __builtin_amdgcn_sched_barrier(0);
      if (FULL && (!WIN || win_inner)) {
        uint32_t *stg = s_stage + (threadIdx.x >> 6) * STG;
        if constexpr (Q8) OutStage<1>::stage_bits(stg, lane, o); else OutStage<OUTS>::stage(stg, lane, o);
        __builtin_amdgcn_fence(__ATOMIC_RELEASE, "wavefront"); __builtin_amdgcn_wave_barrier(); __builtin_amdgcn_fence(__ATOMIC_ACQUIRE, "wavefront");
        if (WIN) OutStage<OUTS>::flush(stg, lane, frame_dst, (size_t)(r - a.out_r0) * win->pitch + (pc0 - win->c0));
        else OutStage<OUTS>::flush(stg, lane, frame_dst, (size_t)(r - a.out_r0) * a.W + pc0);
        __builtin_amdgcn_fence(__ATOMIC_RELEASE, "wavefront"); __builtin_amdgcn_wave_barrier(); __builtin_amdgcn_fence(__ATOMIC_ACQUIRE, "wavefront");
      } else if (WIN) {
        if (lane_on) win_store<OUTS, Q8>(frame_dst, (size_t)(r - a.out_r0) * win->pitch, col0, win->c0, win->c1, o);
      } else {
        if (lane_on) OutStore<OUTS>::store(frame_dst, (size_t)(r - a.out_r0) * a.W + col0, nvalid, o, store_aligned);
      }
      __builtin_amdgcn_sched_barrier(0);
      raw_next = issue_row(min(r + 3, Hm1));
      P = NN; fP = fNN;
      if (GEN) ry = (ry + 1 == a.gen_ph) ? 0u : ry + 1;
    };
    for (uint32_t r = r0, r1d = r1; r < r1d; ++r) {
      uint32_t e_now = r1;
      if (steal_on) {
        if (lane == 0) __hip_atomic_store(&s_tcur[wslot], r, __ATOMIC_RELAXED, __HIP_MEMORY_SCOPE_WORKGROUP);
        e_now = (uint32_t)__hip_atomic_load(reinterpret_cast<uint32_t *>(&s_tdesc[wslot]), __ATOMIC_RELAXED, __HIP_MEMORY_SCOPE_WORKGROUP);
      }
      row_step(P, C, N, fP, fC, fN, r);
      { const RowWin t = P; P = C; C = N; N = t; const bool ft = fP; fP = fC; fC = fN; fN = ft; }
      if (steal_on) r1d = (uint32_t)__builtin_amdgcn_readfirstlane((int)e_now);
    }
  }
  arrive();
  if (queued && (threadIdx.x & 63u) == 0) {
    uint32_t *const arrived = a.task_ctr + kQueueStride;
    if (atomicAdd(arrived, 1u) == n_waves - 1u) {
      __hip_atomic_store(a.task_ctr, 0u, __ATOMIC_RELAXED, __HIP_MEMORY_SCOPE_AGENT);
      __hip_atomic_store(arrived, 0u, __ATOMIC_RELAXED, __HIP_MEMORY_SCOPE_AGENT);
    }
  }
}
template <typename SrcT, bool VEC, int OUT, bool FULL, bool GEN, bool PXG = true, int CM = 0, bool ROT = false>
__global__ __launch_bounds__(1024) void k_fused_bayer(FusedArgs a) { fused_bayer_body<SrcT, VEC, OUT, FULL, GEN, PXG, CM, ROT, false>(a, nullptr); }
template <typename SrcT, bool VEC, int OUT, bool PXG>
__global__ __launch_bounds__(1024) void k_fused_bayer_batch(FusedArgs a, BatchPtrs bp) { fused_bayer_body<SrcT, VEC, OUT, true, false, PXG, 1, false, true>(a, &bp); }
template <typename SrcT, bool VEC, int OUT, bool FULL, bool GEN, bool PXG, int CM>
__global__ __launch_bounds__(1024) void k_fused_bayer_window(FusedArgs a, FusedWindow w) { fused_bayer_body<SrcT, VEC, OUT, FULL, GEN, PXG, CM, false, false, true>(a, nullptr, &w); }

static void fused_task_grid(FusedArgs &a, int num_cus, unsigned &blocks, uint32_t frames = 1, uint32_t waves_per_block = 16);
static bool task_counters_for(TaskQueues *q, hipStream_t s, FusedArgs &a, std::unique_lock<std::mutex> &lk);
static int launch_status() { return hipGetLastError() == hipSuccess ? 0 : -4; }

int launch_demosaic_bayer(const float *src, size_t width, size_t img_height, size_t src_row0, size_t out_row0, size_t out_rows,
                          int xoff, int yoff, const float *gen_cells, int gen_pw, int gen_ph, float *dst4, int num_cus, TaskQueues *queues, hipStream_t s) {
  FusedArgs a;
  std::memset(&a, 0, sizeof(a));
  a.src = src; a.dst = dst4; a.W = (uint32_t)width; a.H = (uint32_t)img_height; a.owidth = width;
  a.row_off = (uint32_t)src_row0; a.out_r0 = (uint32_t)out_row0; a.out_r1 = (uint32_t)(out_row0 + out_rows);
  a.xoff = xoff; a.yoff = yoff; a.range0 = 1.0f; a.inv_range0 = 1.0f;
  a.gen_cells = gen_cells; a.gen_pw = (uint32_t)gen_pw; a.gen_ph = (uint32_t)gen_ph;
  unsigned blocks;
  std::unique_lock<std::mutex> queue_lock;
  (void)task_counters_for(queues, s, a, queue_lock);
  fused_task_grid(a, gen_cells ? num_cus : 2 * (num_cus > 0 ? num_cus : 256), blocks);
  if (gen_cells) {
    if (a.W >= 256u) IPK_LAUNCH((k_fused_bayer<float, true, 3, true, true>), dim3(blocks), dim3(1024), 0, s, a);
    else IPK_LAUNCH((k_fused_bayer<float, true, 3, false, true>), dim3(blocks), dim3(1024), 0, s, a);
  } else {
    if (a.W >= 256u) IPK_LAUNCH((k_fused_bayer<float, true, 3, true, false>), dim3(blocks), dim3(1024), 0, s, a);
    else IPK_LAUNCH((k_fused_bayer<float, true, 3, false, false>), dim3(blocks), dim3(1024), 0, s, a);
  }
  return launch_status();
}

template <typename SrcT, bool VEC, int OUT>
static void launch_fused_t(const FusedArgs &a, unsigned grid, hipStream_t s) {
  const unsigned tpb = 1024;
  const bool common_but_curve = a.fast_ok && a.has_curve && !a.exact_norm && (a.linear != 0) == (OUT == 2) && a.W >= 256u &&
                                std::fabs(a.min0) >= 0x1p-70f && std::fabs(a.min0) <= 0x1p70f;
  const bool common = common_but_curve && a.spline.npoints == 3 && spline3_arith_ok(a.spline);
  const bool common_grid = common_but_curve && a.spline.grid_ok != 0 && a.ori == 0 && !a.gen_cells;
  if (a.ori != 0) {
    if (a.gen_cells) { IPK_LAUNCH((k_fused_bayer<SrcT, sizeof(SrcT) == 4, OUT, true, true, true, true, true>), dim3(grid), dim3(tpb), 0, s, a); return; }
    if (a.px_guard == 0) IPK_LAUNCH((k_fused_bayer<SrcT, sizeof(SrcT) == 4, OUT, true, false, false, true, true>), dim3(grid), dim3(tpb), 0, s, a);
    else IPK_LAUNCH((k_fused_bayer<SrcT, sizeof(SrcT) == 4, OUT, true, false, true, true, true>), dim3(grid), dim3(tpb), 0, s, a);
    return;
  }
  if (a.gen_cells) {
    constexpr bool V = sizeof(SrcT) == 4;
    const char *const tag = a.four ? "four=1" : nullptr;
    if (common) IPK_LAUNCH((k_fused_bayer<SrcT, V, OUT, true, true, true, true>), dim3(grid), dim3(tpb), 0, s, a);
    else if (a.W >= 256u) IPK_LAUNCH_TAG(tag, (k_fused_bayer<SrcT, V, OUT, true, true>), dim3(grid), dim3(tpb), 0, s, a);
    else IPK_LAUNCH_TAG(tag, (k_fused_bayer<SrcT, V, OUT, false, true>), dim3(grid), dim3(tpb), 0, s, a);
    return;
  }
  if constexpr (sizeof(SrcT) == 2) if (a.px_guard == 0 && a.W >= 256u) {
    if (common) IPK_LAUNCH((k_fused_bayer<SrcT, false, OUT, true, false, false, true>), dim3(grid), dim3(tpb), 0, s, a);
    else if (common_grid) IPK_LAUNCH((k_fused_bayer<SrcT, false, OUT, true, false, false, 2>), dim3(grid), dim3(tpb), 0, s, a);
    else IPK_LAUNCH((k_fused_bayer<SrcT, false, OUT, true, false, false, false>), dim3(grid), dim3(tpb), 0, s, a);
    return;
  }
  if (common_grid) {
    if constexpr (sizeof(SrcT) == 4) if (a.px_guard == 0) {
      IPK_LAUNCH((k_fused_bayer<SrcT, true, OUT, true, false, false, 2>), dim3(grid), dim3(tpb), 0, s, a);
      return;
    }
    IPK_LAUNCH((k_fused_bayer<SrcT, sizeof(SrcT) == 4, OUT, true, false, true, 2>), dim3(grid), dim3(tpb), 0, s, a);
    return;
  }
  if (common) {
    if constexpr (sizeof(SrcT) == 4) if (a.px_guard == 0) {
      IPK_LAUNCH((k_fused_bayer<SrcT, true, OUT, true, false, false, true>), dim3(grid), dim3(tpb), 0, s, a);
      return;
    }
    IPK_LAUNCH((k_fused_bayer<SrcT, sizeof(SrcT) == 4, OUT, true, false, true, true>), dim3(grid), dim3(tpb), 0, s, a);
    return;
  }
  if (a.W >= 256u) IPK_LAUNCH((k_fused_bayer<SrcT, VEC, OUT, true, false>), dim3(grid), dim3(tpb), 0, s, a);
  else IPK_LAUNCH((k_fused_bayer<SrcT, VEC, OUT, false, false>), dim3(grid), dim3(tpb), 0, s, a);
}
template <typename SrcT, int OUT>
static void launch_fused_window_t(const FusedArgs &a, const FusedWindow &w, unsigned grid, hipStream_t s) {
  constexpr bool V = sizeof(SrcT) == 4;
  const bool full = w.x1 - w.x0 >= 256u;
  const bool common = full && a.fast_ok && a.has_curve && !a.exact_norm && (a.linear != 0) == (OUT == 2) && std::fabs(a.min0) >= 0x1p-70f &&
                      std::fabs(a.min0) <= 0x1p70f && a.spline.npoints == 3 && spline3_arith_ok(a.spline);
#define IPK_WIN_LAUNCH(FL, G, P, C) IPK_LAUNCH_TAG((a.four ? "four=1" : nullptr), (k_fused_bayer_window<SrcT, V, OUT, FL, G, P, C>), dim3(grid), dim3(1024), 0, s, a, w)
  if (a.gen_cells) {
    if (common) IPK_WIN_LAUNCH(true, true, true, 1);
    else if (full) IPK_WIN_LAUNCH(true, true, true, 0);
    else IPK_WIN_LAUNCH(false, true, true, 0);
  }
  else if (common && a.px_guard == 0) IPK_WIN_LAUNCH(true, false, false, 1);
  else if (common) IPK_WIN_LAUNCH(true, false, true, 1);
  else if (full) IPK_WIN_LAUNCH(true, false, true, 0);
  else IPK_WIN_LAUNCH(false, false, true, 0);
#undef IPK_WIN_LAUNCH
}

constexpr uint32_t kCtrSlots = 1024;
constexpr uint32_t kCtrSlotWords = 2 * kQueueStride;
struct StreamCtr { hipStream_t key; hipStream_t stream; uint32_t slot; uint64_t last_use; };
struct TaskQueues {
  std::mutex mu;
  uint32_t *block = nullptr;
  std::vector<StreamCtr> of;
  uint64_t clock = 0;
};
static std::atomic<bool> g_ctr_disabled{false};
TaskQueues *create_task_queues() {
  TaskQueues *q = new TaskQueues;
  if (hipMalloc(reinterpret_cast<void **>(&q->block), (size_t)kCtrSlots * kCtrSlotWords * sizeof(uint32_t)) != hipSuccess) { delete q; return nullptr; }
  if (hipMemset(q->block, 0, (size_t)kCtrSlots * kCtrSlotWords * sizeof(uint32_t)) != hipSuccess) { (void)hipFree(q->block); delete q; return nullptr; }
  return q;
}
void destroy_task_queues(TaskQueues *q) {
  if (!q) return;
  { std::lock_guard<std::mutex> lk(q->mu); if (q->block) (void)hipFree(q->block); q->block = nullptr; q->of.clear(); }
  delete q;
}
void selftest_task_queue(bool enabled) { g_ctr_disabled.store(!enabled); }
static bool task_counters_for(TaskQueues *q, hipStream_t s, FusedArgs &a, std::unique_lock<std::mutex> &lk) {
  a.task_ctr = nullptr;
  if (!q) return false;
  lk = std::unique_lock<std::mutex>(q->mu);
  if (!q->block || g_ctr_disabled.load()) return false;
  static thread_local char per_thread_key;
  const hipStream_t key = (s == hipStreamPerThread) ? reinterpret_cast<hipStream_t>(&per_thread_key) : s;
  StreamCtr *e = nullptr;
  for (auto &c : q->of) if (c.key == key) { e = &c; break; }
  if (!e) {
    if (q->of.size() < kCtrSlots) {
      q->of.push_back({key, s, (uint32_t)q->of.size(), 0});
      e = &q->of.back();
    } else {
      hipStreamCaptureStatus cap = hipStreamCaptureStatusNone;
      if (hipStreamIsCapturing(s, &cap) != hipSuccess || cap != hipStreamCaptureStatusNone) { (void)hipGetLastError(); return false; }
      StreamCtr *lru = nullptr;
      uint64_t older_than = 0;
      for (int attempt = 0; attempt < 8 && !lru; ++attempt) {
        StreamCtr *cand = nullptr;
        for (auto &c : q->of) if (c.key == c.stream && c.last_use > older_than && (!cand || c.last_use < cand->last_use)) cand = &c;
        if (!cand) break;
        older_than = cand->last_use;
        const hipError_t qs = hipStreamQuery(cand->stream);
        (void)hipGetLastError();
        if (qs != hipErrorNotReady) lru = cand;
      }
      if (!lru) return false;
      lru->key = key; lru->stream = s;
      e = lru;
    }
  }
  e->last_use = ++q->clock;
  a.task_ctr = q->block + (size_t)e->slot * kCtrSlotWords;
  return true;
}

static void fused_task_grid(FusedArgs &a, int num_cus, unsigned &blocks, uint32_t frames, uint32_t waves_per_block) {
  const uint32_t uni = 32u, share_min = frames == 1 ? 128u : 64u;
  const uint32_t grid = (uint32_t)(num_cus > 0 ? num_cus : 256);
  const uint32_t total_waves = grid * waves_per_block;
  const uint32_t w4 = (a.W + 3) / 4;
  a.n_strips = (w4 + 63) / 64;
  a.lc_base = w4 / a.n_strips; a.lc_rem = w4 % a.n_strips;
  const uint32_t nrows = a.out_r1 - a.out_r0;
  const uint64_t share = (uint64_t)nrows * a.n_strips * frames / total_waves;
  if (share >= share_min && a.task_ctr != nullptr) a.n_segs = std::max(1u, nrows / uni);
  else {
    const uint32_t min_rows = kMinTaskRows;
    a.n_segs = std::min(nrows, std::min(std::max(1u, (uint32_t)(total_waves / ((uint64_t)a.n_strips * frames))), std::max(1u, nrows / min_rows)));
  }
  const uint64_t tasks = (uint64_t)a.n_strips * a.n_segs * frames;
  const bool drawn = share >= share_min && a.task_ctr != nullptr;
  const uint64_t per_block = !drawn ? (uint64_t)kSpread : waves_per_block;
  blocks = (unsigned)std::min<uint64_t>(grid, (tasks + per_block - 1) / per_block);
}

int launch_fused_bayer(const FusedLaunch &f, hipStream_t s) {
  FusedArgs a;
  a.src = f.src; a.dst = f.dst; a.W = (uint32_t)f.width; a.H = (uint32_t)f.height; a.owidth = f.owidth;
  a.row_off = (uint32_t)f.row_off; a.out_r0 = (uint32_t)f.out_r0; a.out_r1 = (uint32_t)f.out_r1;
  a.min0 = f.black0; a.range0 = f.white0 - f.black0;
  a.inv_range0 = 1.0f / a.range0;
  a.exact_norm = f.exact_norm;
  a.fast_ok = f.fast_ok;
  a.xoff = f.xoff; a.yoff = f.yoff;
  a.tolab = make_tolab(f.mul4, f.cm12);
  for (int i = 0; i < 9; ++i) a.rgbm.m[i] = f.rgbm9[i];
  a.has_curve = f.has_curve; a.linear = f.linear;
  if (f.has_curve) a.spline = make_spline(*f.spline); else { a.spline.npoints = 0; a.spline.nseg = 0; a.spline.grid_ok = 0; }
  if (f.has_curve && a.spline.npoints == 2) {
    a.spline.npoints = 3; a.spline.nseg = 2;
    a.spline.px[2] = a.spline.px[1]; a.spline.py[2] = a.spline.py[1];
    a.spline.c1[1] = a.spline.c1[0]; a.spline.c2[1] = a.spline.c2[0]; a.spline.c3[1] = a.spline.c3[0];
    a.spline.c1[2] = a.spline.c1[1];
  }
  a.lab_table = reinterpret_cast<const float *>(f.lab_table);
  a.gam_table = reinterpret_cast<const float *>(f.gam_table);
  a.lab_pairs = reinterpret_cast<const LutPair *>(f.lab_pairs); a.gam_pairs = reinterpret_cast<const LutPair *>(f.gam_pairs);
  a.gam_q8 = reinterpret_cast<const Q8Entry *>(f.gam_q8);
  a.gen_cells = f.gen_cells; a.gen_pw = (uint32_t)f.gen_pw; a.gen_ph = (uint32_t)f.gen_ph; a.gen_check = f.gen_check; a.px_guard = f.px_guard;
  a.four = f.four ? 1 : 0;
  if (a.four) {
    if (!a.gen_cells || f.ori != 0 || f.out_type < 0 || f.out_type > 2) return -2;
    a.fast_ok = 0;
  }
  a.ori = f.ori;
  for (int i = 0; i < 4; ++i) a.roles[i] = f.roles[i];
  if (f.ori != 0) {
    const bool common = a.fast_ok && a.has_curve && a.spline.npoints == 3 && spline3_arith_ok(a.spline) && !a.exact_norm && (a.linear != 0) == (f.out_type == 2) && a.W >= 256u &&
                        std::fabs(a.min0) >= 0x1p-70f && std::fabs(a.min0) <= 0x1p70f;
    if (!common || f.ori < 1 || f.ori > 7) return -2;
  }
  if (f.win_c1 != 0) {
    if (f.ori != 0 || f.batch_n > 0 || f.out_type < 0 || f.out_type > 2 || f.win_c0 >= f.win_c1 || f.win_c1 > f.width) return -2;
    FusedWindow w;
    w.c0 = (uint32_t)f.win_c0; w.c1 = (uint32_t)f.win_c1; w.pitch = f.win_c1 - f.win_c0;
    w.x0 = w.c0 & ~3u; w.x1 = std::min(a.W, (w.c1 + 3u) & ~3u);
    std::unique_lock<std::mutex> queue_lock;
    (void)task_counters_for(f.queues, s, a, queue_lock);
    unsigned blocks;
    a.W = w.x1 - w.x0; fused_task_grid(a, f.num_cus, blocks); a.W = (uint32_t)f.width;
    if (!f.src_is_u16) {
      if (f.out_type == 0) launch_fused_window_t<float, 0>(a, w, blocks, s);
      else if (f.out_type == 1) launch_fused_window_t<float, 1>(a, w, blocks, s);
      else launch_fused_window_t<float, 2>(a, w, blocks, s);
    } else {
      if (f.out_type == 0) launch_fused_window_t<uint16_t, 0>(a, w, blocks, s);
      else if (f.out_type == 1) launch_fused_window_t<uint16_t, 1>(a, w, blocks, s);
      else launch_fused_window_t<uint16_t, 2>(a, w, blocks, s);
    }
    return launch_status();
  }

  const bool vec = f.src_is_u16 ? f.src_aligned4 : true;
  if (f.batch_n > 0) {
    const bool common = a.fast_ok && a.has_curve && a.spline.npoints == 3 && spline3_arith_ok(a.spline) && !a.exact_norm && (a.linear != 0) == (f.out_type == 2) && a.W >= 256u &&
                        std::fabs(a.min0) >= 0x1p-70f && std::fabs(a.min0) <= 0x1p70f;
    const bool batchable = common && a.ori == 0 && !a.gen_cells && a.px_guard == 0 && f.batch_n > 1;
    for (int i0 = 0; i0 < f.batch_n; i0 += kBatchMax) {
      const int n = std::min(kBatchMax, f.batch_n - i0);
      if (batchable && n > 1) {
        BatchPtrs bp;
        for (int i = 0; i < n; ++i) { bp.src[i] = f.batch_src[i0 + i]; bp.dst[i] = f.batch_dst[i0 + i]; }
        for (int i = n; i < kBatchMax; ++i) { bp.src[i] = nullptr; bp.dst[i] = nullptr; }
        a.n_frames = (uint32_t)n;
        unsigned grid;
        std::unique_lock<std::mutex> queue_lock;
        (void)task_counters_for(f.queues, s, a, queue_lock);
        fused_task_grid(a, f.num_cus, grid, (uint32_t)n);
#define IPK_BATCH_LAUNCH(T, V, O) IPK_LAUNCH((k_fused_bayer_batch<T, V, O, false>), dim3(grid), dim3(1024), 0, s, a, bp)
        if (!f.src_is_u16) { if (f.out_type == 0) IPK_BATCH_LAUNCH(float, true, 0); else if (f.out_type == 1) IPK_BATCH_LAUNCH(float, true, 1); else IPK_BATCH_LAUNCH(float, true, 2); }
        else { if (f.out_type == 0) IPK_BATCH_LAUNCH(uint16_t, false, 0); else if (f.out_type == 1) IPK_BATCH_LAUNCH(uint16_t, false, 1); else IPK_BATCH_LAUNCH(uint16_t, false, 2); }
#undef IPK_BATCH_LAUNCH
        if (const int rc = launch_status()) return rc;
      } else {
        FusedLaunch one = f;
        one.batch_n = 0;
        for (int i = 0; i < n; ++i) { one.src = f.batch_src[i0 + i]; one.dst = f.batch_dst[i0 + i]; const int rc = launch_fused_bayer(one, s); if (rc) return rc; }
      }
    }
    return 0;
  }
  std::unique_lock<std::mutex> queue_lock;
  (void)task_counters_for(f.queues, s, a, queue_lock);
  unsigned blocks;
  fused_task_grid(a, f.num_cus, blocks);
  if (f.schedule == 1 && a.n_strips * a.n_segs <= (uint32_t)(f.num_cus > 0 ? f.num_cus : 256) * 16u && (a.out_r1 - a.out_r0) / a.n_segs >= IPK_SPLIT_MIN_ROWS) {
    a.n_segs *= 2u; a.task_ctr = nullptr;
  }
  if (f.out_type == 4) {
    if (a.gen_cells || a.ori != 0 || a.W < 256u || a.exact_norm || std::fabs(a.min0) < 0x1p-70f || std::fabs(a.min0) > 0x1p70f) return -2;
    if (!f.src_is_u16) IPK_LAUNCH((k_fused_bayer<float, true, 4, true, false, false, true>), dim3(blocks), dim3(1024), 0, s, a);
    else IPK_LAUNCH((k_fused_bayer<uint16_t, false, 4, true, false, false, true>), dim3(blocks), dim3(1024), 0, s, a);
    return launch_status();
  }
  if (!f.src_is_u16) {
    if (f.out_type == 0) launch_fused_t<float, true, 0>(a, blocks, s);
    else if (f.out_type == 1) launch_fused_t<float, true, 1>(a, blocks, s);
    else launch_fused_t<float, true, 2>(a, blocks, s);
  } else if (vec) {
    if (f.out_type == 0) launch_fused_t<uint16_t, true, 0>(a, blocks, s);
    else if (f.out_type == 1) launch_fused_t<uint16_t, true, 1>(a, blocks, s);
    else launch_fused_t<uint16_t, true, 2>(a, blocks, s);
  } else {
    if (f.out_type == 0) launch_fused_t<uint16_t, false, 0>(a, blocks, s);
    else if (f.out_type == 1) launch_fused_t<uint16_t, false, 1>(a, blocks, s);
    else launch_fused_t<uint16_t, false, 2>(a, blocks, s);
  }
  return launch_status();
}


template <bool TOLAB_ONLY, int NPV = 2>
__device__ __forceinline__ void pointwise_chain_body(const FusedArgs &a, uint64_t npix) {
  constexpr int NP = TOLAB_ONLY ? 1 : NPV, PPL = 2 * NP;
  constexpr uint64_t CH = 64u * PPL;
  __shared__ __attribute__((aligned(16))) LabTab s_lab[kLutPairs + 4];
  __shared__ __attribute__((aligned(16))) GamTab s_gam[TOLAB_ONLY ? 4 : kLutPairs + 4];
  __shared__ __attribute__((aligned(16))) float s_knots[kKnotFloats];
  __shared__ float s_par[32];
  stage_table_direct(s_lab, a.lab_table, a.lab_pairs);
  if (!TOLAB_ONLY) stage_table_direct(s_gam, a.gam_table, a.gam_pairs);
  if (threadIdx.x < 4) s_par[threadIdx.x] = a.tolab.mul[threadIdx.x];
  else if (threadIdx.x < 16) s_par[threadIdx.x] = a.tolab.cm[threadIdx.x - 4];
  else if (threadIdx.x < 25) s_par[threadIdx.x] = a.rgbm.m[threadIdx.x - 16];
  if (threadIdx.x < kSplineMaxKnots) fill_knots(s_knots, a.spline, (int)threadIdx.x);
  __shared__ __attribute__((aligned(16))) float s_grid[TOLAB_ONLY ? 4 : kGridFloats];
  if (!TOLAB_ONLY && a.spline.grid_ok) fill_grid(s_grid, a.spline, (int)threadIdx.x);
  bool arrived = false;
  const uint32_t lane = threadIdx.x & 63u;
  const uint64_t wave = (uint64_t)blockIdx.x * (blockDim.x >> 6) + (threadIdx.x >> 6);
  const uint64_t nwaves = (uint64_t)gridDim.x * (blockDim.x >> 6);
  const uint64_t nchunks = (npix + CH - 1) / CH;
  const float4 *src = reinterpret_cast<const float4 *>(a.src);
  f3 *dst = reinterpret_cast<f3 *>(a.dst);
  for (uint64_t chunk = wave; chunk < nchunks; chunk += nwaves) {
    const uint64_t base = chunk * CH + lane;
    float4 px[PPL];
    #pragma unroll
// ... 477 lines not shown
  return launch_status();
}

struct SelftestOut { unsigned long long bad; unsigned int first_bad; unsigned int pad; };

__device__ __forceinline__ bool same_f32(float a, float b) {
  return (__float_as_uint(a) == __float_as_uint(b)) || (a != a && b != b);
}
__global__ void k_selftest_cdiv(float c, float rc, float rc_lo, int variant, unsigned lo_bits, unsigned hi_bits, int include_special,
                                SelftestOut *out) {
  unsigned long long bad = 0; unsigned first = 0xFFFFFFFFu;
  const unsigned long long total = 1ull << 32, stride = (unsigned long long)gridDim.x * blockDim.x;
  for (unsigned long long i = (unsigned long long)blockIdx.x * blockDim.x + threadIdx.x; i < total; i += stride) {
    const unsigned bits = (unsigned)i, mag = bits & 0x7FFFFFFFu;
    const bool special = mag == 0 || mag >= 0x7F800000u;
    if (special ? !include_special : (mag < lo_bits || mag > hi_bits)) continue;
    const float x = __uint_as_float(bits);
    float q;
    if (variant == 0) q = cdiv_fast(x, c, rc);
    else if (variant == 1) { const float q0 = x * rc; const float r = __builtin_fmaf(-q0, c, x); q = __builtin_fmaf(r, rc, q0); }
    else { const float t = x * rc_lo; q = __builtin_fmaf(x, rc, t); }
    if (!same_f32(q, x / c)) { ++bad; if (bits < first) first = bits; }
  }
  if (bad) { atomicAdd(&out->bad, bad); atomicMin(&out->first_bad, first); }
}
__global__ void k_selftest_fract(SelftestOut *out) {
  unsigned long long bad = 0; unsigned first = 0xFFFFFFFFu;
  const unsigned hi = __float_as_uint(8192.0f);
  for (unsigned long long i = (unsigned long long)blockIdx.x * blockDim.x + threadIdx.x; i <= hi; i += (unsigned long long)gridDim.x * blockDim.x) {
    const float pos = __uint_as_float((unsigned)i);
    if (!same_f32(pos - truncf(pos), __builtin_amdgcn_fractf(pos))) { ++bad; if ((unsigned)i < first) first = (unsigned)i; }
  }
  if (bad) { atomicAdd(&out->bad, bad); atomicMin(&out->first_bad, first); }
}
__global__ void k_selftest_clamp(SelftestOut *out) {
  unsigned long long bad = 0; unsigned first = 0xFFFFFFFFu;
  const unsigned long long total = 1ull << 32, stride = (unsigned long long)gridDim.x * blockDim.x;
  for (unsigned long long i = (unsigned long long)blockIdx.x * blockDim.x + threadIdx.x; i < total; i += stride) {
    const float v = __uint_as_float((unsigned)i);
    const float a = rs_min(rs_max(v, 0.0f), 1.0f), b = __builtin_amdgcn_fmed3f(v, 0.0f, 1.0f);
    if (!(a == b)) { ++bad; if ((unsigned)i < first) first = (unsigned)i; }
  }
  if (bad) { atomicAdd(&out->bad, bad); atomicMin(&out->first_bad, first); }
}
__global__ __launch_bounds__(256) void k_copy_probe(const ipk_f4v *__restrict__ src, ipk_f4v *__restrict__ dst, size_t n16) {
  const size_t base = (size_t)blockIdx.x * 1024 + threadIdx.x;
  ipk_f4v v[4];
  #pragma unroll
  for (int u = 0; u < 4; ++u) if (base + u * 256 < n16) v[u] = __builtin_nontemporal_load(src + base + u * 256);
  #pragma unroll
  for (int u = 0; u < 4; ++u) if (base + u * 256 < n16) __builtin_nontemporal_store(v[u], dst + base + u * 256);
}
constexpr int kMixU = 1;
__global__ __launch_bounds__(256) void k_mix_probe(const ipk_f4v *__restrict__ src, ipk_f4v *__restrict__ dst, size_t n16) {
  constexpr int U = kMixU;
  const size_t base = (size_t)blockIdx.x * (256 * U) + threadIdx.x;
  ipk_f4v v[U];
  #pragma unroll
  for (int u = 0; u < U; ++u) if (base + u * 256 < n16) v[u] = __builtin_nontemporal_load(src + base + u * 256);
  #pragma unroll
  for (int u = 0; u < U; ++u) if (base + u * 256 < n16) {
    ipk_f4v *o = dst + (size_t)blockIdx.x * (768 * U) + u * 768 + threadIdx.x;
    __builtin_nontemporal_store(v[u], o); __builtin_nontemporal_store(v[u], o + 256); __builtin_nontemporal_store(v[u], o + 512);
  }
}
void launch_mix_probe(const void *src, void *dst, size_t src_bytes, hipStream_t s) {
  const size_t n16 = src_bytes / 16, per = 256 * kMixU;
  IPK_LAUNCH(k_mix_probe, dim3((unsigned)std::max<size_t>(1, (n16 + per - 1) / per)), dim3(256), 0, s, reinterpret_cast<const ipk_f4v *>(src), reinterpret_cast<ipk_f4v *>(dst), n16);
}
void launch_copy_probe(const void *src, void *dst, size_t bytes, int, hipStream_t s) {
  const size_t n16 = bytes / 16;
  IPK_LAUNCH(k_copy_probe, dim3((unsigned)std::max<size_t>(1, (n16 + 1023) / 1024)), dim3(256), 0, s, reinterpret_cast<const ipk_f4v *>(src), reinterpret_cast<ipk_f4v *>(dst), n16);
}
__global__ __launch_bounds__(64) void k_clock_probe(unsigned long long *out2, unsigned long long spin_ticks) {
  const unsigned long long c0 = __builtin_amdgcn_s_memtime(), r0 = __builtin_amdgcn_s_memrealtime();
  unsigned long long r1 = r0;
  while (r1 - r0 < spin_ticks) { __builtin_amdgcn_s_sleep(32); r1 = __builtin_amdgcn_s_memrealtime(); }
  const unsigned long long c1 = __builtin_amdgcn_s_memtime();
  if (threadIdx.x == 0) { out2[0] = c1 - c0; out2[1] = r1 - r0; }
}
void launch_clock_probe(void *out2_dev, unsigned long long spin_ticks, hipStream_t s) {
  IPK_LAUNCH(k_clock_probe, dim3(1), dim3(64), 0, s, reinterpret_cast<unsigned long long *>(out2_dev), spin_ticks);
}
__global__ void k_selftest_spline3(SplineDev sp, SelftestOut *out) {
  __shared__ __attribute__((aligned(16))) float s_knots[kKnotFloats];
  __shared__ __attribute__((aligned(16))) float s_grid[kGridFloats];
  if (threadIdx.x < kSplineMaxKnots) fill_knots(s_knots, sp, (int)threadIdx.x);
  if (sp.grid_ok) fill_grid(s_grid, sp, (int)threadIdx.x);
  __syncthreads();
  unsigned long long bad = 0; unsigned first = 0xFFFFFFFFu;
  const unsigned long long total = 1ull << 32, stride = (unsigned long long)gridDim.x * blockDim.x;
  for (unsigned long long i = (unsigned long long)blockIdx.x * blockDim.x + threadIdx.x; i < total; i += stride) {
    const float v = __uint_as_float((unsigned)i);
    const float want = spline_interpolate_lds(s_knots, sp.npoints, sp.nseg, v), got = sp.grid_ok ? spline_interpolate_grid(sp, s_grid, v) : spline_interpolate_3a(sp, s_knots, v);
    const bool same = __float_as_uint(want) == __float_as_uint(got) || (want != want && got != got) || (sp.grid_ok && v != v);
    if (!same) { ++bad; if ((unsigned)i < first) first = (unsigned)i; }
  }
  if (bad) { atomicAdd(&out->bad, bad); atomicMin(&out->first_bad, first); }
}
__global__ void k_selftest_quant8(SelftestOut *out, int variant) {
  unsigned long long bad = 0; unsigned first = 0xFFFFFFFFu;
  const unsigned long long total = 1ull << 32, stride = (unsigned long long)gridDim.x * blockDim.x;
  for (unsigned long long i = (unsigned long long)blockIdx.x * blockDim.x + threadIdx.x; i < total; i += stride) {
    const float v = __uint_as_float((unsigned)i);
    const uint32_t a = output8bit_literal(v);
    const float p = v * 256.0f;
    uint32_t b;
    if (variant == 0) b = __builtin_amdgcn_cvt_pk_u8_f32(p, 0u, 0u);
    else if (variant == 1) b = __builtin_amdgcn_cvt_pk_u8_f32(floorf(p), 0u, 0u);
    else b = min(f32_as_u32_sat(p), 255u);
    if (a != b) { ++bad; if ((unsigned)i < first) first = (unsigned)i; }
  }
  if (bad) { atomicAdd(&out->bad, bad); atomicMin(&out->first_bad, first); }
}
__device__ __forceinline__ uint32_t q8_literal(const LutPair *__restrict__ pairs, float c) { return (uint32_t)output8bit(lut_interp(pairs, c)); }
__global__ void k_build_q8(const LutPair *__restrict__ pairs, Q8Entry *__restrict__ out) {
  const uint32_t i = blockIdx.x * blockDim.x + threadIdx.x;
  if (i >= (uint32_t)kLutPairs) return;
  auto first_with_key = [&](uint32_t key) {
    uint32_t lo = 0u, hi = 0x3F800001u;
    while (lo < hi) { const uint32_t mid = lo + (hi - lo) / 2u; if (f32_as_u32_sat(__uint_as_float(mid) * kLutMaxF) >= key) hi = mid; else lo = mid + 1u; }
    return lo;
  };
  const uint32_t b0 = first_with_key(i), b1 = first_with_key(i + 1u);
  Q8Entry e; e.k = 0u; e.t = __builtin_inff();
  if (b0 < b1) {
    e.k = q8_literal(pairs, __uint_as_float(b0));
    if (q8_literal(pairs, __uint_as_float(b1 - 1u)) != e.k) {
      uint32_t lo = b0, hi = b1 - 1u;
      while (lo < hi) { const uint32_t mid = lo + (hi - lo) / 2u; if (q8_literal(pairs, __uint_as_float(mid)) > e.k) hi = mid; else lo = mid + 1u; }
      e.t = __uint_as_float(lo);
    }
  }
  out[i] = e;
}
void launch_build_q8(const void *gam_pairs, void *q8_out, hipStream_t s) {
  IPK_LAUNCH(k_build_q8, dim3(kLutPairs / 256), dim3(256), 0, s, reinterpret_cast<const LutPair *>(gam_pairs), reinterpret_cast<Q8Entry *>(q8_out));
}
__global__ void k_selftest_q8(const LutPair *__restrict__ pairs, const Q8Entry *__restrict__ q8, SelftestOut *out) {
  unsigned long long bad = 0; unsigned first = 0xFFFFFFFFu;
  const unsigned long long total = 1ull << 32, stride = (unsigned long long)gridDim.x * blockDim.x;
  for (unsigned long long i = (unsigned long long)blockIdx.x * blockDim.x + threadIdx.x; i < total; i += stride) {
    const float x = __uint_as_float((unsigned)i);
    const uint32_t a = (uint32_t)output8bit_literal(gamma_sample(pairs, x));
    const uint32_t b = q8_sample(q8, __builtin_amdgcn_fmed3f(x, 0.0f, 1.0f));
    if (a != b) { ++bad; if ((unsigned)i < first) first = (unsigned)i; }
  }
  if (bad) { atomicAdd(&out->bad, bad); atomicMin(&out->first_bad, first); }
}
__global__ void k_selftest_quant16(SelftestOut *out) {
  unsigned long long bad = 0; unsigned first = 0xFFFFFFFFu;
  const unsigned long long total = 1ull << 32, stride = (unsigned long long)gridDim.x * blockDim.x;
  for (unsigned long long i = (unsigned long long)blockIdx.x * blockDim.x + threadIdx.x; i < total; i += stride) {
    const float v = __uint_as_float((unsigned)i);
    const uint32_t a = output16bit_literal(v);
    const uint32_t w = output16bit_x2(v, -v), w2 = output16bit_x2(0.25f, v);
    if ((w & 0xFFFFu) != a || (w2 >> 16) != a || (w2 & 0xFFFFu) != 16384u) { ++bad; if ((unsigned)i < first) first = (unsigned)i; }
  }
  if (bad) { atomicAdd(&out->bad, bad); atomicMin(&out->first_bad, first); }
}
int launch_selftest_quant16(void *out_dev, hipStream_t s) { IPK_LAUNCH(k_selftest_quant16, dim3(256 * 8), dim3(256), 0, s, reinterpret_cast<SelftestOut *>(out_dev)); return 0; }
int launch_selftest_q8(const void *gam_pairs, const void *q8, void *out_dev, hipStream_t s) {
  IPK_LAUNCH(k_selftest_q8, dim3(256 * 8), dim3(256), 0, s, reinterpret_cast<const LutPair *>(gam_pairs), reinterpret_cast<const Q8Entry *>(q8), reinterpret_cast<SelftestOut *>(out_dev));
  return 0;
}
__global__ void k_selftest_cbrt(const float *__restrict__ in, float *__restrict__ out, size_t n, int variant) {
  for (size_t i = (size_t)blockIdx.x * blockDim.x + threadIdx.x; i < n; i += (size_t)gridDim.x * blockDim.x) {
    const float x = in[i];
    out[i] = variant == 0 ? cbrtf_glibc(x) : (variant == 1 ? cbrtf_glibc_sel(x) : cbrtf_glibc_1to2(x));
  }
}
template <bool PXG>
__device__ __forceinline__ void selftest_lab_slot(const LutPair *__restrict__ s_lab, const float (&v)[1], float (&f)[1], const int cm) {
  constexpr int NS = 1;
#include "ipk_lab_slots.inc"
}
__global__ __launch_bounds__(256) void k_selftest_lab_slot(const float *__restrict__ in, float *__restrict__ out, size_t n, int variant, const LutPair *__restrict__ lab_pairs) {
  __shared__ __attribute__((aligned(16))) LutPair lab[kLutPairs + 4];
  load_lut_pairs(lab, lab_pairs);
  __syncthreads();
  for (size_t i = (size_t)blockIdx.x * blockDim.x + threadIdx.x; i < n; i += (size_t)gridDim.x * blockDim.x) {
    const float v[1] = {in[i]};
    float f[1];
    if (variant == 3) selftest_lab_slot<false>(lab, v, f, 1);
    else if (variant == 4) selftest_lab_slot<true>(lab, v, f, 0);
    else f[0] = lab_lookup(lab, v[0]);
    out[i] = f[0];
  }
}

int launch_selftest_cdiv(float c, int variant, unsigned lo_bits, unsigned hi_bits, int include_special, void *out_dev, hipStream_t s) {
  const float rc = 1.0f / c;
  const float rc_lo = (float)(1.0 / (double)c - (double)rc);
  IPK_LAUNCH(k_selftest_cdiv, dim3(256 * 8), dim3(256), 0, s, c, rc, rc_lo, variant, lo_bits, hi_bits, include_special,
                     reinterpret_cast<SelftestOut *>(out_dev));
  return 0;
}
int launch_selftest_spline3(const SplineHost &h, void *out_dev, hipStream_t s) {
  SplineDev d = make_spline(h);
  if (d.npoints == 2) {
    d.npoints = 3; d.nseg = 2; d.px[2] = d.px[1]; d.py[2] = d.py[1];
    d.c1[1] = d.c1[0]; d.c2[1] = d.c2[0]; d.c3[1] = d.c3[0]; d.c1[2] = d.c1[1];
  }
  if (!d.grid_ok && (d.npoints != 3 || !spline3_arith_ok(d))) return -2;
  IPK_LAUNCH(k_selftest_spline3, dim3(256 * 8), dim3(256), 0, s, d, reinterpret_cast<SelftestOut *>(out_dev));
  return 0;
}
int launch_selftest_fract(void *out_dev, hipStream_t s) { IPK_LAUNCH(k_selftest_fract, dim3(256 * 8), dim3(256), 0, s, reinterpret_cast<SelftestOut *>(out_dev)); return 0; }
int launch_selftest_clamp(void *out_dev, hipStream_t s) { IPK_LAUNCH(k_selftest_clamp, dim3(256 * 8), dim3(256), 0, s, reinterpret_cast<SelftestOut *>(out_dev)); return 0; }
int launch_selftest_quant8(void *out_dev, int variant, hipStream_t s) { IPK_LAUNCH(k_selftest_quant8, dim3(256 * 8), dim3(256), 0, s, reinterpret_cast<SelftestOut *>(out_dev), variant); return 0; }
int launch_selftest_cbrt(const float *in, float *out, size_t n, int variant, const void *lab_pairs, hipStream_t s) {
  if (variant >= 3) IPK_LAUNCH(k_selftest_lab_slot, dim3(256 * 8), dim3(256), 0, s, in, out, n, variant, reinterpret_cast<const LutPair *>(lab_pairs));
  else IPK_LAUNCH(k_selftest_cbrt, dim3(256 * 8), dim3(256), 0, s, in, out, n, variant);
  return 0;
}

}
```

### imagepipe_amd/csrc/ipk_launch.hpp

```cpp
#pragma once
#include <hip/hip_runtime_api.h>
#include <cstddef>
#include <cstdint>
#include "ipk_host.hpp"

namespace ipk {

typedef Spline SplineHost;

struct TaskQueues;
TaskQueues *create_task_queues();
void destroy_task_queues(TaskQueues *q);

template <typename T>
void launch_gofloat_cfa(const T *src, size_t owidth, size_t x, size_t y, size_t w, size_t h, float black0, float white0,
                        float *dst, hipStream_t s);
template <typename T>
void launch_gofloat_mono(const T *src, size_t owidth, size_t x, size_t y, size_t w, size_t h, float black0, float white0,
                         float *dst4, hipStream_t s);
template <typename T>
void launch_gofloat_rgb(const T *src, size_t owidth, size_t x, size_t y, size_t w, size_t h, const float *black4, const float *white4,
                        float *dst4, hipStream_t s);
void launch_gofloat_other_u8(const uint8_t *src, size_t owidth, size_t x, size_t y, size_t w, size_t h,
                             const void *gamma_reverse_pairs, float *dst4, hipStream_t s);
void launch_gofloat_other_u16(const uint16_t *src, size_t owidth, size_t x, size_t y, size_t w, size_t h, float *dst4, hipStream_t s);

void launch_demosaic_full(const float *src, size_t width, size_t img_height, size_t src_row0, size_t out_row0, size_t out_rows,
                          const uint32_t *lookups_dev, float *dst4, hipStream_t s);

int launch_demosaic_bayer(const float *src, size_t width, size_t img_height, size_t src_row0, size_t out_row0, size_t out_rows,
                          int xoff, int yoff, const float *gen_cells, int gen_pw, int gen_ph, float *dst4, int num_cus, TaskQueues *queues, hipStream_t s);
void selftest_task_queue(bool enabled);
void launch_log_enable(bool on);
size_t launch_log_read(char *buf, size_t cap);

template <typename T>
void launch_transform_buffer(const T *src, size_t width, size_t height, int64_t tlx, int64_t tly, int64_t trx, int64_t try_,
                             int64_t blx, int64_t bly, size_t nwidth, size_t nheight, size_t components,
                             const uint8_t *cfa48_dev, T *dst, hipStream_t s);

void launch_raster_scale_down(const void *src, int src_is_u16, size_t owidth, size_t x, size_t y, size_t width, size_t height,
                              size_t nwidth, size_t nheight, const void *gamma_reverse_pairs, float *dst4, hipStream_t s);
template <typename T>
void launch_raw_scaled_demosaic(const T *src, size_t owidth, size_t x, size_t y, size_t width, size_t height, float black0, float white0, int norm_fast, int has_fourth_colour,
                                size_t nwidth, size_t nheight, const uint8_t *cfa48_dev, int pattern_width, int pattern_height, float *dst4, hipStream_t s,
                                size_t band_src_row0 = 0, size_t band_out_row0 = 0, size_t band_out_rows = 0);

void launch_tolab(const float *src4, size_t npix, const float *mul4, const float *cm12, const void *lab_pairs, float *dst3,
                  int num_cus, hipStream_t s);
void launch_basecurve(const float *src3, size_t npix, const SplineHost &sp, float *dst3, int num_cus, hipStream_t s);
void launch_fromlab(const float *src3, size_t npix, const float *m9, float *dst3, int num_cus, hipStream_t s);
void launch_gamma(const float *src, size_t n, const void *gam_pairs, float *dst, int num_cus, hipStream_t s);
template <typename T>
void launch_rotate(const T *src3, size_t owidth, size_t oheight, int64_t base_offset_px, int64_t x_step_px, int64_t y_step_px,
                   T *dst3, hipStream_t s);
void launch_output8(const float *src, size_t n, uint8_t *dst, int num_cus, hipStream_t s);
void launch_output16(const float *src, size_t n, uint16_t *dst, int num_cus, hipStream_t s);
void launch_chan_8_to_16(const uint8_t *src, size_t n, uint16_t *dst, int num_cus, hipStream_t s);
void launch_chan_16_to_8(const uint16_t *src, size_t n, uint8_t *dst, int num_cus, hipStream_t s);

struct FusedLaunch {
  const void *src; void *dst;
  bool src_is_u16, src_aligned4;
  size_t width, height, owidth;
  size_t row_off, out_r0, out_r1;
  float black0, white0;
  int exact_norm;
  int fast_ok;
  int xoff, yoff;
  const float *mul4, *cm12, *rgbm9;
  int has_curve, linear;
  const SplineHost *spline;
  int out_type;
  const void *lab_table, *gam_table;
  const void *lab_pairs, *gam_pairs;
  const void *gam_q8;
  int px_guard;
  const float *gen_cells; int gen_pw, gen_ph, gen_check;
  int four = 0;
  int num_cus;
  int schedule;
  TaskQueues *queues;
  int ori;
  int roles[4];
  int batch_n; const void *const *batch_src; void *const *batch_dst;
  size_t win_c0 = 0, win_c1 = 0;
};
int launch_fused_bayer(const FusedLaunch &f, hipStream_t s);
struct ResampleWindow { size_t row0, col0, rows, cols; };
int launch_fused_resample(const FusedLaunch &f, const ResamplePlan &plan, size_t nwidth, size_t nheight, const uint32_t *lookups_dev, hipStream_t s,
                          const ResampleWindow *win = nullptr);
constexpr size_t kRotate1MaxTransposedRows = 65535u * 64u;
template <typename T>
void launch_rotate1(const T *src, size_t owidth, size_t oheight, int64_t base_offset, int64_t x_step, int64_t y_step, T *dst, hipStream_t s);
int launch_pointwise_chain(const FusedLaunch &f, size_t npix, hipStream_t s);
int launch_tolab_fast(const FusedLaunch &f, size_t npix, hipStream_t s);
int launch_chain_quantised(const FusedLaunch &f, size_t npix, hipStream_t s);
int launch_raster_chain(const FusedLaunch &f, size_t npix, int src_is_u16, const void *gamma_reverse_pairs, hipStream_t s);

int launch_selftest_cdiv(float c, int variant, unsigned lo_bits, unsigned hi_bits, int include_special, void *out_dev, hipStream_t s);
void launch_copy_probe(const void *src, void *dst, size_t bytes, int num_cus, hipStream_t s);
void launch_mix_probe(const void *src, void *dst, size_t src_bytes, hipStream_t s);
void launch_clock_probe(void *out2_dev, unsigned long long spin_ticks, hipStream_t s);
int launch_selftest_spline3(const SplineHost &h, void *out_dev, hipStream_t s);
int launch_selftest_fract(void *out_dev, hipStream_t s);
int launch_selftest_clamp(void *out_dev, hipStream_t s);
int launch_selftest_quant8(void *out_dev, int variant, hipStream_t s);
int launch_selftest_quant16(void *out_dev, hipStream_t s);
void launch_build_q8(const void *gam_pairs, void *q8_out, hipStream_t s);
int launch_selftest_q8(const void *gam_pairs, const void *q8, void *out_dev, hipStream_t s);
int launch_selftest_cbrt(const float *in, float *out, size_t n, int variant, const void *lab_pairs, hipStream_t s);

}
```

### include/imagepipe_amd.h

```cpp
#ifndef IMAGEPIPE_AMD_H
#define IMAGEPIPE_AMD_H

#include <stddef.h>
#include <stdint.h>

#ifdef __cplusplus
extern "C" {
#endif

#define IPK_API __attribute__((visibility("default")))

typedef enum {
  IPK_OK = 0,
  IPK_NOOP = 1,
  IPK_ERR_NOT_INIT = -1,
  IPK_ERR_INVALID = -2,
  IPK_ERR_HIP = -3,
  IPK_ERR_NO_DEVICE = -4,
  IPK_ERR_UNSUPPORTED = -5,
  IPK_ERR_NOMEM = -6
} ipk_status;

typedef enum {
  IPK_OR_NORMAL = 0, IPK_OR_HFLIP = 1, IPK_OR_ROT180 = 2, IPK_OR_VFLIP = 3, IPK_OR_TRANSPOSE = 4,
// ... 217 lines not shown
IPK_API int ipk_host_pipeline_run_region(const ipk_pipeline_desc *d, const void *src, size_t x, size_t y, size_t w, size_t h, void *dst,
                                         int out_type, int *windowed);
IPK_API int ipk_host_pipeline_run_batch(const ipk_pipeline_desc *d, const void *const *srcs, void *const *dsts, size_t n,
                                        int out_type, int *used_fused);
IPK_API int ipk_pipeline_run_batch(const ipk_pipeline_desc *d, const void *const *srcs, void *const *dsts, size_t n, int out_type,
                                   int *used_fused, void *stream);
IPK_API int ipk_pipeline_run_batch_multi(const ipk_pipeline_desc *d, const void *const *srcs, void *const *dsts, size_t n, int out_type,
                                         int *used_fused);
IPK_API int ipk_devices_sync(void);
IPK_API int ipk_host_pipeline_run_batch_multi(const ipk_pipeline_desc *d, const void *const *srcs, void *const *dsts, size_t n,
                                              int out_type, int *used_fused);
IPK_API void *ipk_host_alloc(size_t bytes);
IPK_API void ipk_host_free(void *p);


IPK_API int ipk_pipeline_hashes(const ipk_pipeline_desc *d, int out_type, uint64_t source_id, uint8_t *out256);

typedef struct ipk_cache ipk_cache;
IPK_API int ipk_cache_new(size_t max_bytes, ipk_cache **out);
IPK_API int ipk_cache_free(ipk_cache *cache);
IPK_API int ipk_cache_clear(ipk_cache *cache);
IPK_API int ipk_cache_contains(const ipk_cache *cache, const uint8_t *key32);
IPK_API int ipk_cache_stats(const ipk_cache *cache, size_t *bytes, size_t *entries, uint64_t *hits, uint64_t *misses, uint64_t *evictions);
IPK_API int ipk_cache_get(ipk_cache *cache, const uint8_t *key32, const float **data, size_t *width, size_t *height,
                          size_t *colors, int *monochrome);

IPK_API int ipk_pipeline_run_cached(const ipk_pipeline_desc *d, const void *src, uint64_t source_id, ipk_cache *cache,
                                    int out_type, void *dst, int *ops_run, int *used_fused, void *stream);


typedef struct { size_t out_row0, out_rows, src_row0, src_rows; } ipk_band;

IPK_API int ipk_band_plan(size_t height, int nranks, int cfa_period, ipk_band *bands);
IPK_API int ipk_band_plan_scaled(size_t height, size_t nheight, int nranks, ipk_band *bands);
IPK_API int ipk_raw_scaled_demosaic_band(const void *src, int src_type, size_t owidth, size_t x, size_t width, size_t height,
                                         float black0, float white0, const char *cfa, size_t nwidth, size_t nheight,
                                         const ipk_band *band, float *dst4, void *stream);

typedef struct ipk_comm ipk_comm;
#define IPK_COMM_ID_BYTES 128
IPK_API int ipk_comm_unique_id(uint8_t *id128);
IPK_API int ipk_comm_init_rccl(const uint8_t *id128, int rank, int nranks, ipk_comm **out);
typedef int (*ipk_exchange_fn)(void *ctx, int send_peer, const void *send, size_t send_bytes, int recv_peer, void *recv, size_t recv_bytes);
IPK_API int ipk_comm_init_host(int rank, int nranks, ipk_exchange_fn exchange, void *ctx, ipk_comm **out);
IPK_API int ipk_comm_free(ipk_comm *comm);
IPK_API int ipk_comm_info(const ipk_comm *comm, int *rank, int *nranks, int *transport);
IPK_API int ipk_band_exchange_halo(ipk_comm *comm, void *slab, size_t row_bytes, const ipk_band *bands, void *stream);
IPK_API int ipk_host_band_exchange_halo(ipk_comm *comm, void *slab, size_t row_bytes, const ipk_band *bands);
IPK_API int ipk_band_gather(ipk_comm *comm, void *frame, size_t out_row_bytes, const ipk_band *bands, int root, void *stream);
IPK_API int ipk_host_band_gather(ipk_comm *comm, void *frame, size_t out_row_bytes, const ipk_band *bands, int root);
IPK_API int ipk_band_gather_begin(ipk_comm *comm, void *frame, size_t out_row_bytes, const ipk_band *bands, int root, void *after_stream);
IPK_API int ipk_comm_wait(ipk_comm *comm, void *stream);
IPK_API int ipk_comm_selftest(ipk_comm *comm);

IPK_API int ipk_host_gofloat_cfa_u16(const uint16_t *src, size_t owidth, size_t oheight, size_t x, size_t y, size_t width, size_t height,
                                     float black0, float white0, float *dst);
IPK_API int ipk_host_gofloat_cfa_f32(const float *src, size_t owidth, size_t oheight, size_t x, size_t y, size_t width, size_t height,
                                     float black0, float white0, float *dst);
IPK_API int ipk_host_demosaic_full(const float *src, size_t width, size_t height, const char *cfa, float *dst4);
IPK_API int ipk_host_transform_buffer_f32(const float *src, size_t width, size_t height,
                                          int64_t tlx, int64_t tly, int64_t trx, int64_t try_, int64_t blx, int64_t bly,
                                          size_t nwidth, size_t nheight, size_t components, const char *cfa, float *dst);
IPK_API int ipk_host_tolab(const float *src4, size_t width, size_t height, int monochrome,
                           const float *wb_coeffs, const float *cam_to_xyz_normalized, float *dst3);
IPK_API int ipk_host_basecurve(const float *src3, size_t width, size_t height, float exposure,
                               const float *points, int npoints, float *dst3);
IPK_API int ipk_host_fromlab(const float *src3, size_t width, size_t height, float *dst3);
IPK_API int ipk_host_gamma(const float *src, size_t width, size_t height, size_t colors, int linear, float *dst);
IPK_API int ipk_host_rotate_buffer(const float *src3, size_t width, size_t height, int orientation,
                                   float *dst3, size_t *out_width, size_t *out_height);
IPK_API int ipk_host_output8bit(const float *src, size_t n, uint8_t *dst);
IPK_API int ipk_host_output16bit(const float *src, size_t n, uint16_t *dst);
IPK_API int ipk_host_raw_to_srgb(const ipk_fused_params *p, const void *src, void *dst);

IPK_API int ipk_selftest_cdiv(float c, int variant, float lo, float hi, int include_special,
                              uint64_t *n_bad, uint32_t *first_bad_bits);
IPK_API int ipk_selftest_lut_weight(uint64_t *n_bad, uint32_t *first_bad_bits);
IPK_API int ipk_selftest_clamp01(uint64_t *n_bad, uint32_t *first_bad_bits);
IPK_API int ipk_copy_probe(const void *src, void *dst, size_t bytes, void *stream);
IPK_API int ipk_mix_probe(const void *src, void *dst, size_t src_bytes, void *stream);
IPK_API int ipk_clock_probe(uint64_t *out2_dev, uint32_t spin_us, void *stream);
IPK_API int ipk_stream_probe(const ipk_fused_params *p, const void *src, void *dst, void *stream);
IPK_API int ipk_selftest_spline3(float exposure, const float *points, int npoints, uint64_t *n_bad, uint32_t *first_bad_bits);
IPK_API int ipk_selftest_quant8(int variant, uint64_t *n_bad, uint32_t *first_bad_bits);
IPK_API int ipk_selftest_q8(uint64_t *n_bad, uint32_t *first_bad_bits);
IPK_API int ipk_selftest_quant16(uint64_t *n_bad, uint32_t *first_bad_bits);
IPK_API int ipk_selftest_cbrtf(const float *in, float *out, size_t n, int variant, void *stream);
IPK_API int ipk_selftest_task_queue(int enabled);
IPK_API int ipk_selftest_launch_log(int enabled);
IPK_API size_t ipk_selftest_launch_log_read(char *buf, size_t cap);
IPK_API int ipk_selftest_cache_put(ipk_cache *cache, const uint8_t *key32, size_t bytes);
IPK_API int ipk_selftest_sha256(const void *data, size_t n, uint8_t *out32);

#ifdef __cplusplus
}
#endif
#endif
```

Baseline: 231,500.

## Trim spline end clamp via med3 and halve f32 output staging LDS

```diff
diff --git a/bindings/rust/imagepipe_amd_sys.rs b/bindings/rust/imagepipe_amd_sys.rs
--- a/bindings/rust/imagepipe_amd_sys.rs
+++ b/bindings/rust/imagepipe_amd_sys.rs
@@ -273,6 +273,8 @@
   pub fn ipk_clock_probe(out2_dev: *mut u64, spin_us: u32, stream: *mut c_void) -> c_int;
   pub fn ipk_stream_probe(p: *const IpkFusedParams, src: *const c_void, dst: *mut c_void, stream: *mut c_void) -> c_int;
   pub fn ipk_selftest_spline3(exposure: f32, points: *const f32, npoints: c_int, n_bad: *mut u64, first_bad_bits: *mut u32) -> c_int;
+  pub fn ipk_selftest_spline3_clamp(exposure: f32, points: *const f32, npoints: c_int, n_bad: *mut u64, first_bad_bits: *mut u32) -> c_int;
+  pub fn ipk_curve_end_clamp_ok(exposure: f32, points: *const f32, npoints: c_int, ok: *mut c_int) -> c_int;
   pub fn ipk_selftest_quant8(variant: c_int, n_bad: *mut u64, first_bad_bits: *mut u32) -> c_int;
   pub fn ipk_selftest_q8(n_bad: *mut u64, first_bad_bits: *mut u32) -> c_int;
   pub fn ipk_selftest_quant16(n_bad: *mut u64, first_bad_bits: *mut u32) -> c_int;
diff --git a/imagepipe_amd/_lib.py b/imagepipe_amd/_lib.py
--- a/imagepipe_amd/_lib.py
+++ b/imagepipe_amd/_lib.py
@@ -179,6 +179,8 @@
     "ipk_clock_probe": (C.c_int, [_vp, C.c_uint32, _vp]),
     "ipk_stream_probe": (C.c_int, [C.POINTER(FusedParams), _vp, _vp, _vp]),
     "ipk_selftest_spline3": (C.c_int, [C.c_float, _fp, C.c_int, C.POINTER(C.c_uint64), C.POINTER(C.c_uint32)]),
+    "ipk_selftest_spline3_clamp": (C.c_int, [C.c_float, _fp, C.c_int, C.POINTER(C.c_uint64), C.POINTER(C.c_uint32)]),
+    "ipk_curve_end_clamp_ok": (C.c_int, [C.c_float, _fp, C.c_int, C.POINTER(C.c_int)]),
     "ipk_selftest_quant8": (C.c_int, [C.c_int, C.POINTER(C.c_uint64), C.POINTER(C.c_uint32)]),
     "ipk_selftest_q8": (C.c_int, [C.POINTER(C.c_uint64), C.POINTER(C.c_uint32)]),
     "ipk_selftest_quant16": (C.c_int, [C.POINTER(C.c_uint64), C.POINTER(C.c_uint32)]),
diff --git a/imagepipe_amd/csrc/ipk_api.cpp b/imagepipe_amd/csrc/ipk_api.cpp
--- a/imagepipe_amd/csrc/ipk_api.cpp
+++ b/imagepipe_amd/csrc/ipk_api.cpp
@@ -1272,6 +1272,22 @@
   if (ipk::launch_selftest_spline3(sp, dev, nullptr) != 0) { (void)hipFree(dev); return fail(IPK_ERR_UNSUPPORTED, "the kernels keep the select form for this curve"); }
   HIPCHK(hipGetLastError());
   return selftest_collect(dev, n_bad, first_bad_bits);
+}
+int ipk_selftest_spline3_clamp(float exposure, const float *points, int npoints, uint64_t *n_bad, uint32_t *first_bad_bits) {
+  REQUIRE_INIT();
+  if (!n_bad || (npoints > 0 && !points)) return fail(IPK_ERR_INVALID, "bad selftest arguments");
+  ipk::Spline sp; int rc = build_curve(exposure, points, npoints, sp); if (rc) return rc;
+  void *dev; rc = selftest_alloc(&dev); if (rc) return rc;
+  if (ipk::launch_selftest_spline3_clamp(sp, dev, nullptr) != 0) { (void)hipFree(dev); return fail(IPK_ERR_UNSUPPORTED, "the kernels keep the select form for this curve"); }
+  HIPCHK(hipGetLastError());
+  return selftest_collect(dev, n_bad, first_bad_bits);
+}
+int ipk_curve_end_clamp_ok(float exposure, const float *points, int npoints, int *ok) {
+  if (!ok || (npoints > 0 && !points)) return fail(IPK_ERR_INVALID, "bad arguments");
+  ipk::Spline sp; int rc = build_curve(exposure, points, npoints, sp); if (rc) return rc;
+  ipk::spline_pad3(sp);
+  *ok = ipk::curve_end_clamp_ok(sp) ? 1 : 0;
+  return IPK_OK;
 }
 int ipk_selftest_quant16(uint64_t *n_bad, uint32_t *first_bad_bits) {
   REQUIRE_INIT();
diff --git a/imagepipe_amd/csrc/ipk_device.hpp b/imagepipe_amd/csrc/ipk_device.hpp
--- a/imagepipe_amd/csrc/ipk_device.hpp
+++ b/imagepipe_amd/csrc/ipk_device.hpp
@@ -244,7 +244,27 @@
   return spline_poly(py[i], c1[i], c2[i], c3[i], val - px[i]);
 }
 
+#ifndef IPK_TRIM_CLAMP
+#define IPK_TRIM_CLAMP 1
+#endif
 __device__ __forceinline__ float spline_interpolate_3a(const SplineDev &s, const float *__restrict__ lds_knots, float val) {
+  const float x0 = s.px[0], x1 = s.px[1], x2 = s.px[2];
+#if IPK_TRIM_CLAMP
+  const float v1 = __builtin_amdgcn_fmed3f(val, x0, x2);
+#else
+  const float v1 = fmaxf(val, x0);
+#endif
+  const bool up = v1 >= x1;
+  const float *rec = lds_knots + kKnotSegRec + (up ? 8 : 0);
+  const float4 q = *reinterpret_cast<const float4 *>(rec);
+  const float r = spline_poly(q.y, q.z, q.w, rec[4], v1 - q.x);
+#if IPK_TRIM_CLAMP
+  return r;
+#else
+  return (val >= x2) ? s.py[2] : r;
+#endif
+}
+__device__ __forceinline__ float spline_interpolate_3s(const SplineDev &s, const float *__restrict__ lds_knots, float val) {
   const float x0 = s.px[0], x1 = s.px[1], x2 = s.px[2];
   const float v1 = fmaxf(val, x0);
   const bool up = v1 >= x1;
diff --git a/imagepipe_amd/csrc/ipk_host.hpp b/imagepipe_amd/csrc/ipk_host.hpp
--- a/imagepipe_amd/csrc/ipk_host.hpp
+++ b/imagepipe_amd/csrc/ipk_host.hpp
@@ -359,6 +359,24 @@
     return true;
   }
 };
+template <typename S>
+inline void spline_pad3(S &d) {
+  if (d.npoints != 2) return;
+  d.npoints = 3; d.nseg = 2; d.px[2] = d.px[1]; d.py[2] = d.py[1];
+  d.c1[1] = d.c1[0]; d.c2[1] = d.c2[0]; d.c3[1] = d.c3[0]; d.c1[2] = d.c1[1];
+}
+template <typename S>
+inline bool curve_end_clamp_ok(const S &d) {
+  if (d.npoints != 3 || d.nseg != 2) return false;
+  for (int i = 0; i < 3; ++i) if (!std::isfinite(d.px[i]) || !std::isfinite(d.py[i])) return false;
+  if (!(std::isfinite(d.c1[1]) && std::isfinite(d.c2[1]) && std::isfinite(d.c3[1]))) return false;
+  if (!(d.px[0] <= d.px[1] && d.px[1] <= d.px[2])) return false;
+  const float diff = d.px[2] - d.px[1];
+  const float r = d.py[1] + d.c1[1] * diff + d.c2[1] * diff * diff + d.c3[1] * diff * diff * diff;
+  uint32_t rb, yb;
+  std::memcpy(&rb, &r, 4); std::memcpy(&yb, &d.py[2], 4);
+  return rb == yb;
+}
 
 inline void orientation_to_flips(int o, bool &transpose, bool &fx, bool &fy) {
   static const bool t[9][3] = {{0,0,0},{0,1,0},{0,1,1},{0,0,1},{1,0,0},{1,0,1},{1,1,1},{1,1,0},{0,0,0}};
diff --git a/imagepipe_amd/csrc/ipk_kernels.hip b/imagepipe_amd/csrc/ipk_kernels.hip
--- a/imagepipe_amd/csrc/ipk_kernels.hip
+++ b/imagepipe_amd/csrc/ipk_kernels.hip
@@ -1055,6 +1055,12 @@
   }
   return true;
 }
+#ifndef IPK_TRIM_GAMPAIR
+#define IPK_TRIM_GAMPAIR 1
+#endif
+static bool spline3_common_ok(const SplineDev &d) {
+  return d.npoints == 3 && spline3_arith_ok(d) && (IPK_TRIM_CLAMP == 0 || curve_end_clamp_ok(d));
+}
 static bool spline_grid_ok(const SplineDev &d, float &scale) {
   if (d.npoints < 4 || d.npoints > kSplineMaxKnots || d.nseg != d.npoints - 1) return false;
   for (int i = 0; i < d.npoints; ++i) {
@@ -1777,6 +1783,24 @@
     (void)g;
   }
 };
+struct OutStageHalfF32 {
+  static __device__ __forceinline__ void stage(uint32_t *stg, uint32_t lane, uint32_t h, const PixOut o[4]) {
+    if ((lane >> 5) == h) OutStage<0>::stage(stg, lane & 31u, o);
+  }
+  static __device__ __forceinline__ void flush(const uint32_t *stg, uint32_t lane, uint32_t h, void *dst, size_t pix) {
+    const float4 *s = reinterpret_cast<const float4 *>(stg);
+    typedef float f4a __attribute__((ext_vector_type(4), aligned(4)));
+    f4a *gn = reinterpret_cast<f4a *>(reinterpret_cast<float *>(dst) + pix * 3 + 384u * h);
+    const float4 q0 = s[lane];
+    f4a v0; v0.x = q0.x; v0.y = q0.y; v0.z = q0.z; v0.w = q0.w;
+    __builtin_nontemporal_store(v0, gn + lane);
+    if (lane < 32u) {
+      const float4 q1 = s[64 + lane];
+      f4a v1; v1.x = q1.x; v1.y = q1.y; v1.z = q1.z; v1.w = q1.w;
+      __builtin_nontemporal_store(v1, gn + 64 + lane);
+    }
+  }
+};
 template <> struct OutStage<1> {
   static __device__ __forceinline__ void stage_bits(uint32_t *stg, uint32_t lane, const PixOut o[4]) {
     auto B = [](float f) { return __float_as_uint(f); };
@@ -1866,7 +1890,8 @@
   constexpr bool GUARD_NORM = sizeof(SrcT) == 4 && !DEMO;
   typedef typename std::conditional<GEN, float, LabTab>::type LabT;
   constexpr bool Q8 = OUTS == 1 && FULL && !GEN && !DEMO && !SKEL;
-  typedef typename std::conditional<Q8, Q8Entry, typename std::conditional<GEN || OUTS == 0, float, GamTab>::type>::type GamT;
+  constexpr bool GPAIR = IPK_TRIM_GAMPAIR != 0 && OUTS == 0 && FULL && !GEN && !PXG && !DEMO && !SKEL;
+  typedef typename std::conditional<Q8, Q8Entry, typename std::conditional<GEN || (OUTS == 0 && !GPAIR), float, GamTab>::type>::type GamT;
   __shared__ __attribute__((aligned(16))) LabT s_lab[DEMO ? 4 : kLutPairs + 4];
   __shared__ __attribute__((aligned(16))) GamT s_gam[DEMO ? 4 : kLutPairs + 4];
   if (!DEMO) {
@@ -1880,7 +1905,7 @@
   constexpr bool FOUR_CAPABLE = GEN && CM == 0 && !ROT && !BATCH && !DEMO && !SKEL;
   float *e4 = nullptr;
   if constexpr (FOUR_CAPABLE) { __shared__ float s_e4[4 * 1024]; e4 = s_e4 + threadIdx.x; }
-  constexpr int STG = DEMO ? 1024 : (OUTS == 0 ? 768 : (OUTS == 1 ? 192 : 384));
+  constexpr int STG = DEMO ? 1024 : (OUTS == 0 ? (GPAIR ? 384 : 768) : (OUTS == 1 ? 192 : 384));
   __shared__ __attribute__((aligned(16))) uint32_t s_stage[FULL ? 16 * STG : 4];
   if (threadIdx.x < 4) s_par[threadIdx.x] = a.tolab.mul[threadIdx.x];
   else if (threadIdx.x < 16) s_par[threadIdx.x] = a.tolab.cm[threadIdx.x - 4];
@@ -2205,11 +2230,22 @@
       __builtin_amdgcn_sched_barrier(0);
       if (FULL && (!WIN || win_inner)) {
         uint32_t *stg = s_stage + (threadIdx.x >> 6) * STG;
+        if constexpr (GPAIR) {
+          const size_t pix = WIN ? (size_t)(r - a.out_r0) * win->pitch + (pc0 - win->c0) : (size_t)(r - a.out_r0) * a.W + pc0;
+          #pragma unroll
+          for (uint32_t h = 0; h < 2u; ++h) {
+            OutStageHalfF32::stage(stg, lane, h, o);
+            __builtin_amdgcn_fence(__ATOMIC_RELEASE, "wavefront"); __builtin_amdgcn_wave_barrier(); __builtin_amdgcn_fence(__ATOMIC_ACQUIRE, "wavefront");
+            OutStageHalfF32::flush(stg, lane, h, frame_dst, pix);
+            __builtin_amdgcn_fence(__ATOMIC_RELEASE, "wavefront"); __builtin_amdgcn_wave_barrier(); __builtin_amdgcn_fence(__ATOMIC_ACQUIRE, "wavefront");
+          }
+        } else {
         if constexpr (Q8) OutStage<1>::stage_bits(stg, lane, o); else OutStage<OUTS>::stage(stg, lane, o);
         __builtin_amdgcn_fence(__ATOMIC_RELEASE, "wavefront"); __builtin_amdgcn_wave_barrier(); __builtin_amdgcn_fence(__ATOMIC_ACQUIRE, "wavefront");
         if (WIN) OutStage<OUTS>::flush(stg, lane, frame_dst, (size_t)(r - a.out_r0) * win->pitch + (pc0 - win->c0));
         else OutStage<OUTS>::flush(stg, lane, frame_dst, (size_t)(r - a.out_r0) * a.W + pc0);
         __builtin_amdgcn_fence(__ATOMIC_RELEASE, "wavefront"); __builtin_amdgcn_wave_barrier(); __builtin_amdgcn_fence(__ATOMIC_ACQUIRE, "wavefront");
+        }
       } else if (WIN) {
         if (lane_on) win_store<OUTS, Q8>(frame_dst, (size_t)(r - a.out_r0) * win->pitch, col0, win->c0, win->c1, o);
       } else {
@@ -2278,7 +2314,7 @@
   const unsigned tpb = 1024;
   const bool common_but_curve = a.fast_ok && a.has_curve && !a.exact_norm && (a.linear != 0) == (OUT == 2) && a.W >= 256u &&
                                 std::fabs(a.min0) >= 0x1p-70f && std::fabs(a.min0) <= 0x1p70f;
-  const bool common = common_but_curve && a.spline.npoints == 3 && spline3_arith_ok(a.spline);
+  const bool common = common_but_curve && a.spline.npoints == 3 && spline3_common_ok(a.spline);
   const bool common_grid = common_but_curve && a.spline.grid_ok != 0 && a.ori == 0 && !a.gen_cells;
   if (a.ori != 0) {
     if (a.gen_cells) { IPK_LAUNCH((k_fused_bayer<SrcT, sizeof(SrcT) == 4, OUT, true, true, true, true, true>), dim3(grid), dim3(tpb), 0, s, a); return; }
@@ -2324,7 +2360,7 @@
   constexpr bool V = sizeof(SrcT) == 4;
   const bool full = w.x1 - w.x0 >= 256u;
   const bool common = full && a.fast_ok && a.has_curve && !a.exact_norm && (a.linear != 0) == (OUT == 2) && std::fabs(a.min0) >= 0x1p-70f &&
-                      std::fabs(a.min0) <= 0x1p70f && a.spline.npoints == 3 && spline3_arith_ok(a.spline);
+                      std::fabs(a.min0) <= 0x1p70f && a.spline.npoints == 3 && spline3_common_ok(a.spline);
 #define IPK_WIN_LAUNCH(FL, G, P, C) IPK_LAUNCH_TAG((a.four ? "four=1" : nullptr), (k_fused_bayer_window<SrcT, V, OUT, FL, G, P, C>), dim3(grid), dim3(1024), 0, s, a, w)
   if (a.gen_cells) {
     if (common) IPK_WIN_LAUNCH(true, true, true, 1);
@@ -2449,7 +2485,7 @@
   a.ori = f.ori;
   for (int i = 0; i < 4; ++i) a.roles[i] = f.roles[i];
   if (f.ori != 0) {
-    const bool common = a.fast_ok && a.has_curve && a.spline.npoints == 3 && spline3_arith_ok(a.spline) && !a.exact_norm && (a.linear != 0) == (f.out_type == 2) && a.W >= 256u &&
+    const bool common = a.fast_ok && a.has_curve && a.spline.npoints == 3 && spline3_common_ok(a.spline) && !a.exact_norm && (a.linear != 0) == (f.out_type == 2) && a.W >= 256u &&
                         std::fabs(a.min0) >= 0x1p-70f && std::fabs(a.min0) <= 0x1p70f;
     if (!common || f.ori < 1 || f.ori > 7) return -2;
   }
@@ -2476,7 +2512,7 @@
 
   const bool vec = f.src_is_u16 ? f.src_aligned4 : true;
   if (f.batch_n > 0) {
-    const bool common = a.fast_ok && a.has_curve && a.spline.npoints == 3 && spline3_arith_ok(a.spline) && !a.exact_norm && (a.linear != 0) == (f.out_type == 2) && a.W >= 256u &&
+    const bool common = a.fast_ok && a.has_curve && a.spline.npoints == 3 && spline3_common_ok(a.spline) && !a.exact_norm && (a.linear != 0) == (f.out_type == 2) && a.W >= 256u &&
                         std::fabs(a.min0) >= 0x1p-70f && std::fabs(a.min0) <= 0x1p70f;
     const bool batchable = common && a.ori == 0 && !a.gen_cells && a.px_guard == 0 && f.batch_n > 1;
     for (int i0 = 0; i0 < f.batch_n; i0 += kBatchMax) {
@@ -3120,7 +3156,7 @@
 void launch_clock_probe(void *out2_dev, unsigned long long spin_ticks, hipStream_t s) {
   IPK_LAUNCH(k_clock_probe, dim3(1), dim3(64), 0, s, reinterpret_cast<unsigned long long *>(out2_dev), spin_ticks);
 }
-__global__ void k_selftest_spline3(SplineDev sp, SelftestOut *out) {
+__global__ void k_selftest_spline3(SplineDev sp, SelftestOut *out, int clamp) {
   __shared__ __attribute__((aligned(16))) float s_knots[kKnotFloats];
   __shared__ __attribute__((aligned(16))) float s_grid[kGridFloats];
   if (threadIdx.x < kSplineMaxKnots) fill_knots(s_knots, sp, (int)threadIdx.x);
@@ -3130,8 +3166,8 @@
   const unsigned long long total = 1ull << 32, stride = (unsigned long long)gridDim.x * blockDim.x;
   for (unsigned long long i = (unsigned long long)blockIdx.x * blockDim.x + threadIdx.x; i < total; i += stride) {
     const float v = __uint_as_float((unsigned)i);
-    const float want = spline_interpolate_lds(s_knots, sp.npoints, sp.nseg, v), got = sp.grid_ok ? spline_interpolate_grid(sp, s_grid, v) : spline_interpolate_3a(sp, s_knots, v);
-    const bool same = __float_as_uint(want) == __float_as_uint(got) || (want != want && got != got) || (sp.grid_ok && v != v);
+    const float want = spline_interpolate_lds(s_knots, sp.npoints, sp.nseg, v), got = clamp ? spline_interpolate_3a(sp, s_knots, v) : (sp.grid_ok ? spline_interpolate_grid(sp, s_grid, v) : spline_interpolate_3s(sp, s_knots, v));
+    const bool same = __float_as_uint(want) == __float_as_uint(got) || (want != want && got != got) || (!clamp && sp.grid_ok && v != v);
     if (!same) { ++bad; if ((unsigned)i < first) first = (unsigned)i; }
   }
   if (bad) { atomicAdd(&out->bad, bad); atomicMin(&out->first_bad, first); }
@@ -3241,7 +3277,15 @@
     d.c1[1] = d.c1[0]; d.c2[1] = d.c2[0]; d.c3[1] = d.c3[0]; d.c1[2] = d.c1[1];
   }
   if (!d.grid_ok && (d.npoints != 3 || !spline3_arith_ok(d))) return -2;
-  IPK_LAUNCH(k_selftest_spline3, dim3(256 * 8), dim3(256), 0, s, d, reinterpret_cast<SelftestOut *>(out_dev));
+  IPK_LAUNCH(k_selftest_spline3, dim3(256 * 8), dim3(256), 0, s, d, reinterpret_cast<SelftestOut *>(out_dev), 0);
+  return 0;
+}
+int launch_selftest_spline3_clamp(const SplineHost &h, void *out_dev, hipStream_t s) {
+  SplineDev d = make_spline(h);
+  spline_pad3(d);
+  d.grid_ok = 0;
+  if (d.npoints != 3 || !spline3_arith_ok(d) || !curve_end_clamp_ok(d)) return -2;
+  IPK_LAUNCH(k_selftest_spline3, dim3(256 * 8), dim3(256), 0, s, d, reinterpret_cast<SelftestOut *>(out_dev), 1);
   return 0;
 }
 int launch_selftest_fract(void *out_dev, hipStream_t s) { IPK_LAUNCH(k_selftest_fract, dim3(256 * 8), dim3(256), 0, s, reinterpret_cast<SelftestOut *>(out_dev)); return 0; }
diff --git a/imagepipe_amd/csrc/ipk_launch.hpp b/imagepipe_amd/csrc/ipk_launch.hpp
--- a/imagepipe_amd/csrc/ipk_launch.hpp
+++ b/imagepipe_amd/csrc/ipk_launch.hpp
@@ -103,6 +103,7 @@
 void launch_mix_probe(const void *src, void *dst, size_t src_bytes, hipStream_t s);
 void launch_clock_probe(void *out2_dev, unsigned long long spin_ticks, hipStream_t s);
 int launch_selftest_spline3(const SplineHost &h, void *out_dev, hipStream_t s);
+int launch_selftest_spline3_clamp(const SplineHost &h, void *out_dev, hipStream_t s);
 int launch_selftest_fract(void *out_dev, hipStream_t s);
 int launch_selftest_clamp(void *out_dev, hipStream_t s);
 int launch_selftest_quant8(void *out_dev, int variant, hipStream_t s);
diff --git a/include/imagepipe_amd.h b/include/imagepipe_amd.h
--- a/include/imagepipe_amd.h
+++ b/include/imagepipe_amd.h
@@ -323,6 +323,8 @@
 IPK_API int ipk_clock_probe(uint64_t *out2_dev, uint32_t spin_us, void *stream);
 IPK_API int ipk_stream_probe(const ipk_fused_params *p, const void *src, void *dst, void *stream);
 IPK_API int ipk_selftest_spline3(float exposure, const float *points, int npoints, uint64_t *n_bad, uint32_t *first_bad_bits);
+IPK_API int ipk_selftest_spline3_clamp(float exposure, const float *points, int npoints, uint64_t *n_bad, uint32_t *first_bad_bits);
+IPK_API int ipk_curve_end_clamp_ok(float exposure, const float *points, int npoints, int *ok);
 IPK_API int ipk_selftest_quant8(int variant, uint64_t *n_bad, uint32_t *first_bad_bits);
 IPK_API int ipk_selftest_q8(uint64_t *n_bad, uint32_t *first_bad_bits);
 IPK_API int ipk_selftest_quant16(uint64_t *n_bad, uint32_t *first_bad_bits);
```

Measured after the change: 231,700 (median of 2 runs). About the same (+0.1%).
